# Codes4Fun/moshi.cpp

Measured on AMD Instinct MI355X. Metric: audio frames/sec (12.5 Hz target) moshika-7B q4_k decode, higher is better.
Workload: dtype q4_K weights x q8_K activations (int8 dot, f32 accumulate); bf16 KV; f32 elsewhere; 1 GPU; moshi-sts --bench loop: mimi encode + Temporal step + 8 Depth steps + mimi decode, moshika q4_k, 1 audio stream per GPU, greedy, ctx capacity 3000; context_fill_start=0, parallelism=1 GPU, device= (gfx950:sramecc+:xnack-)

## Files before the change

### include/ggml-backend.h

```cpp
#pragma once

#include "ggml.h"

#ifdef __cplusplus
extern "C" {
#endif

typedef struct ggml_backend_buffer_type * ggml_backend_buffer_type_t;
typedef struct ggml_backend_buffer      * ggml_backend_buffer_t;
typedef struct ggml_backend             * ggml_backend_t;
typedef struct ggml_backend_reg         * ggml_backend_reg_t;
typedef struct ggml_backend_device      * ggml_backend_dev_t;

enum ggml_backend_dev_type {
    GGML_BACKEND_DEVICE_TYPE_CPU,
    GGML_BACKEND_DEVICE_TYPE_GPU,
    GGML_BACKEND_DEVICE_TYPE_ACCEL,
};

struct ggml_backend_dev_caps {
    bool async;
    bool host_buffer;
    bool buffer_from_host_ptr;
    bool events;
};

struct ggml_backend_dev_props {
    const char * name;
    const char * description;
    size_t memory_free;
    size_t memory_total;
    enum ggml_backend_dev_type type;
    struct ggml_backend_dev_caps caps;
};

GGML_API void   ggml_backend_load_all(void);
GGML_API size_t ggml_backend_reg_count(void);
GGML_API ggml_backend_reg_t ggml_backend_reg_get(size_t index);
GGML_API const char * ggml_backend_reg_name(ggml_backend_reg_t reg);
GGML_API void * ggml_backend_reg_get_proc_address(ggml_backend_reg_t reg, const char * name);

GGML_API size_t             ggml_backend_dev_count(void);
GGML_API ggml_backend_dev_t ggml_backend_dev_get(size_t index);
GGML_API ggml_backend_dev_t ggml_backend_dev_by_name(const char * name);
GGML_API ggml_backend_dev_t ggml_backend_dev_by_type(enum ggml_backend_dev_type type);
GGML_API const char *       ggml_backend_dev_name(ggml_backend_dev_t device);
GGML_API const char *       ggml_backend_dev_description(ggml_backend_dev_t device);
GGML_API enum ggml_backend_dev_type ggml_backend_dev_type(ggml_backend_dev_t device);
GGML_API void               ggml_backend_dev_memory(ggml_backend_dev_t device, size_t * free, size_t * total);
GGML_API void               ggml_backend_dev_get_props(ggml_backend_dev_t device, struct ggml_backend_dev_props * props);
GGML_API ggml_backend_reg_t ggml_backend_dev_backend_reg(ggml_backend_dev_t device);
GGML_API ggml_backend_t     ggml_backend_dev_init(ggml_backend_dev_t device, const char * params);

GGML_API ggml_backend_t ggml_backend_init_by_name(const char * name, const char * params);
GGML_API ggml_backend_t ggml_backend_init_by_type(enum ggml_backend_dev_type type, const char * params);
GGML_API ggml_backend_t ggml_backend_init_best(void);

GGML_API const char *       ggml_backend_name(ggml_backend_t backend);
GGML_API void               ggml_backend_free(ggml_backend_t backend);
GGML_API ggml_backend_dev_t ggml_backend_get_device(ggml_backend_t backend);
GGML_API void               ggml_backend_synchronize(ggml_backend_t backend);

typedef void (*ggml_backend_set_n_threads_t)(ggml_backend_t backend, int n_threads);

GGML_API ggml_backend_buffer_t ggml_backend_alloc_ctx_tensors(struct ggml_context * ctx, ggml_backend_t backend);
GGML_API void    ggml_backend_buffer_free    (ggml_backend_buffer_t buffer);
GGML_API size_t  ggml_backend_buffer_get_size(ggml_backend_buffer_t buffer);
GGML_API void *  ggml_backend_buffer_get_base(ggml_backend_buffer_t buffer);
GGML_API const char * ggml_backend_buffer_name(ggml_backend_buffer_t buffer);
GGML_API void    ggml_backend_buffer_clear   (ggml_backend_buffer_t buffer, uint8_t value);
GGML_API bool    ggml_backend_buffer_is_host (ggml_backend_buffer_t buffer);

GGML_API void ggml_backend_tensor_set   (      struct ggml_tensor * tensor, const void * data, size_t offset, size_t size);
GGML_API void ggml_backend_tensor_get   (const struct ggml_tensor * tensor,       void * data, size_t offset, size_t size);
GGML_API void ggml_backend_tensor_get_async(ggml_backend_t backend, const struct ggml_tensor * tensor, void * data, size_t offset, size_t size);
typedef struct ggml_backend_event * ggml_backend_event_t;
GGML_API ggml_backend_event_t ggml_backend_event_new(ggml_backend_dev_t device);
GGML_API void ggml_backend_event_free(ggml_backend_event_t event);
GGML_API void ggml_backend_event_record(ggml_backend_event_t event, ggml_backend_t backend);
GGML_API void ggml_backend_event_synchronize(ggml_backend_event_t event);
GGML_API void ggml_backend_event_wait(ggml_backend_t backend, ggml_backend_event_t event);
GGML_API void ggml_backend_tensor_memset(      struct ggml_tensor * tensor, uint8_t value,     size_t offset, size_t size);
GGML_API void ggml_backend_tensor_copy  (struct ggml_tensor * src, struct ggml_tensor * dst);

GGML_API enum ggml_status ggml_backend_graph_compute(ggml_backend_t backend, struct ggml_cgraph * cgraph);
GGML_API bool ggml_backend_supports_op(ggml_backend_t backend, const struct ggml_tensor * op);

struct ggml_mi355x_stats {
    int64_t graphs_computed;
    int64_t graph_replays;
    int64_t kernels_in_last_plan;
    int64_t fused_nodes_in_last_plan;
    int64_t nodes_in_last_plan;
    int64_t uploads_batched;
    int64_t chained_matvecs_in_last_plan;
    int64_t attention_folds_planned;
    int64_t chain_step_programs_in_last_plan;
    int64_t vq_levels_chained_in_last_plan;
    int64_t attn_block_launches_in_last_plan;
    int64_t attn_block_jobs_in_last_plan;
    int64_t generic_attention_nodes_in_last_plan;
    int64_t ring_copy_launches_in_last_plan;
    int64_t ring_copy_jobs_in_last_plan;
};
GGML_API void ggml_backend_mi355x_get_stats(ggml_backend_t backend, struct ggml_mi355x_stats * stats);
struct ggml_mi355x_kernel_profile {
    double  seconds;
    int64_t launches;
    int64_t bytes;
    double  variant_seconds[3];
    int64_t variant_launches[3];
    int64_t variant_bytes[3];
    double  chain_seconds;
    int64_t chain_launches;
    int64_t chain_bytes;
    int64_t chain_phases;
};
GGML_API void ggml_backend_mi355x_get_kernel_profile(ggml_backend_t backend, struct ggml_mi355x_kernel_profile * out);
GGML_API void ggml_backend_mi355x_set_flags(ggml_backend_t backend, int flags);
GGML_API void ggml_backend_mi355x_set_capture(ggml_backend_t backend, int enabled);
GGML_API void * ggml_backend_mi355x_get_stream(ggml_backend_t backend);
GGML_API void ggml_backend_mi355x_make_current(ggml_backend_t backend);
GGML_API ggml_backend_t ggml_backend_mi355x_init_stream(ggml_backend_t base);

#ifdef __cplusplus
}
#endif
```

### moshi.cpp_amd/__init__.py

```python
import ctypes as C
import os

_HERE = os.path.dirname(os.path.abspath(__file__))
LIB_PATH = os.environ.get("MI355X_LIB") or os.path.join(_HERE, "libggml-mi355x.so")
HOT_LIB_PATH = os.environ.get("MI355X_HOT_LIB") or os.path.join(os.path.dirname(LIB_PATH), "libmoshi-hot.so")

GGML_MAX_DIMS, GGML_MAX_SRC, GGML_MAX_NAME = 4, 10, 64

F32, F16, Q4_0, Q8_0, Q4_K, Q8_K, I32, I64, BF16 = 0, 1, 2, 8, 12, 15, 26, 27, 30
TYPE_NAMES = {F32: "f32", F16: "f16", Q4_0: "q4_0", Q8_0: "q8_0", Q4_K: "q4_K", Q8_K: "q8_K", I32: "i32", I64: "i64", BF16: "bf16"}
DEV_CPU, DEV_GPU = 0, 1


class Tensor(C.Structure):
    pass


Tensor._fields_ = [
    ("type", C.c_int),
    ("buffer", C.c_void_p),
    ("ne", C.c_int64 * GGML_MAX_DIMS),
    ("nb", C.c_size_t * GGML_MAX_DIMS),
    ("op", C.c_int),
    ("op_params", C.c_int32 * 16),
    ("flags", C.c_int32),
    ("src", C.POINTER(Tensor) * GGML_MAX_SRC),
    ("view_src", C.POINTER(Tensor)),
    ("view_offs", C.c_size_t),
    ("data", C.c_void_p),
    ("name", C.c_char * GGML_MAX_NAME),
    ("extra", C.c_void_p),
    ("padding", C.c_char * 8),
]
TP = C.POINTER(Tensor)


class InitParams(C.Structure):
    _fields_ = [("mem_size", C.c_size_t), ("mem_buffer", C.c_void_p), ("no_alloc", C.c_bool)]


class DevProps(C.Structure):
    _fields_ = [("name", C.c_char_p), ("description", C.c_char_p), ("memory_free", C.c_size_t), ("memory_total", C.c_size_t),
                ("type", C.c_int), ("caps", C.c_bool * 4)]


class Stats(C.Structure):
    _fields_ = [(n, C.c_int64) for n in ("graphs_computed", "graph_replays", "kernels_in_last_plan",
                                         "fused_nodes_in_last_plan", "nodes_in_last_plan", "uploads_batched", "chained_matvecs_in_last_plan",
                                         "attention_folds_planned", "chain_step_programs_in_last_plan", "vq_levels_chained_in_last_plan",
                                         "attn_block_launches_in_last_plan", "attn_block_jobs_in_last_plan", "generic_attention_nodes_in_last_plan",
                                         "ring_copy_launches_in_last_plan", "ring_copy_jobs_in_last_plan")]


class KernelProfile(C.Structure):
    _fields_ = [("seconds", C.c_double), ("launches", C.c_int64), ("bytes", C.c_int64),
                ("variant_seconds", C.c_double * 3), ("variant_launches", C.c_int64 * 3), ("variant_bytes", C.c_int64 * 3),
                ("chain_seconds", C.c_double), ("chain_launches", C.c_int64), ("chain_bytes", C.c_int64), ("chain_phases", C.c_int64)]


class GGUFInitParams(C.Structure):
    _fields_ = [("no_alloc", C.c_bool), ("ctx", C.POINTER(C.c_void_p))]


P, I, L, Z, F, B, S = C.c_void_p, C.c_int, C.c_int64, C.c_size_t, C.c_float, C.c_bool, C.c_char_p

SIGNATURES = {
    "ggml_time_ms": (L, []), "ggml_time_us": (L, []), "ggml_time_init": (None, []),
    "ggml_type_name": (S, [I]), "ggml_op_name": (S, [I]), "ggml_op_desc": (S, [TP]), "ggml_status_to_string": (S, [I]),
    "ggml_blck_size": (L, [I]), "ggml_type_size": (Z, [I]), "ggml_row_size": (Z, [I, L]), "ggml_is_quantized": (B, [I]),
    "ggml_nelements": (L, [TP]), "ggml_nrows": (L, [TP]), "ggml_nbytes": (Z, [TP]), "ggml_element_size": (Z, [TP]),
    "ggml_n_dims": (I, [TP]), "ggml_is_contiguous": (B, [TP]), "ggml_is_transposed": (B, [TP]), "ggml_is_permuted": (B, [TP]),
    "ggml_are_same_shape": (B, [TP, TP]),
    "ggml_fp16_to_fp32": (F, [C.c_uint16]), "ggml_fp32_to_fp16": (C.c_uint16, [F]),
    "ggml_bf16_to_fp32": (F, [C.c_uint16]), "ggml_fp32_to_bf16": (C.c_uint16, [F]),
    "ggml_init": (P, [InitParams]), "ggml_reset": (None, [P]), "ggml_free": (None, [P]), "ggml_used_mem": (Z, [P]),
    "ggml_get_no_alloc": (B, [P]), "ggml_set_no_alloc": (None, [P, B]),
    "ggml_tensor_overhead": (Z, []), "ggml_graph_overhead": (Z, []), "ggml_graph_overhead_custom": (Z, [Z, B]),
    "ggml_new_tensor": (TP, [P, I, I, C.POINTER(L)]), "ggml_new_tensor_1d": (TP, [P, I, L]), "ggml_new_tensor_2d": (TP, [P, I, L, L]),
    "ggml_new_tensor_3d": (TP, [P, I, L, L, L]), "ggml_new_tensor_4d": (TP, [P, I, L, L, L, L]),
    "ggml_dup_tensor": (TP, [P, TP]), "ggml_view_tensor": (TP, [P, TP]),
    "ggml_get_first_tensor": (TP, [P]), "ggml_get_next_tensor": (TP, [P, TP]), "ggml_get_tensor": (TP, [P, S]),
    "ggml_get_name": (S, [TP]), "ggml_set_name": (TP, [TP, S]), "ggml_format_name": (TP, [TP, S]),
    "ggml_set_input": (None, [TP]), "ggml_set_output": (None, [TP]), "ggml_get_unary_op": (I, [TP]),
    "ggml_dup": (TP, [P, TP]), "ggml_add": (TP, [P, TP, TP]), "ggml_add_inplace": (TP, [P, TP, TP]), "ggml_sub": (TP, [P, TP, TP]),
    "ggml_sub_inplace": (TP, [P, TP, TP]), "ggml_mul_inplace": (TP, [P, TP, TP]), "ggml_div_inplace": (TP, [P, TP, TP]),
    "ggml_mul": (TP, [P, TP, TP]), "ggml_div": (TP, [P, TP, TP]), "ggml_neg": (TP, [P, TP]),
    "ggml_scale": (TP, [P, TP, F]), "ggml_scale_inplace": (TP, [P, TP, F]), "ggml_clamp": (TP, [P, TP, F, F]),
    "ggml_sum": (TP, [P, TP]), "ggml_sum_rows": (TP, [P, TP]), "ggml_argmax": (TP, [P, TP]),
    "ggml_argsort": (TP, [P, TP, I]), "ggml_argsort_top_k": (TP, [P, TP, I]), "ggml_top_k": (TP, [P, TP, I]),
    "ggml_arange": (TP, [P, F, F, F]), "ggml_repeat": (TP, [P, TP, TP]), "ggml_repeat_4d": (TP, [P, TP, L, L, L, L]),
    "ggml_concat": (TP, [P, TP, TP, I]), "ggml_pad": (TP, [P, TP, I, I, I, I]),
    "ggml_silu": (TP, [P, TP]), "ggml_gelu": (TP, [P, TP]), "ggml_elu": (TP, [P, TP]),
    "ggml_norm": (TP, [P, TP, F]), "ggml_rms_norm": (TP, [P, TP, F]), "ggml_mul_mat": (TP, [P, TP, TP]),
    "ggml_soft_max": (TP, [P, TP]), "ggml_soft_max_ext": (TP, [P, TP, TP, F, F]),
    "ggml_cast": (TP, [P, TP, I]), "ggml_cpy": (TP, [P, TP, TP]), "ggml_cont": (TP, [P, TP]),
    "ggml_reshape_1d": (TP, [P, TP, L]), "ggml_reshape_2d": (TP, [P, TP, L, L]), "ggml_reshape_3d": (TP, [P, TP, L, L, L]),
    "ggml_reshape_4d": (TP, [P, TP, L, L, L, L]),
    "ggml_view_1d": (TP, [P, TP, L, Z]), "ggml_view_2d": (TP, [P, TP, L, L, Z, Z]), "ggml_view_3d": (TP, [P, TP, L, L, L, Z, Z, Z]),
    "ggml_view_4d": (TP, [P, TP, L, L, L, L, Z, Z, Z, Z]),
    "ggml_permute": (TP, [P, TP, I, I, I, I]), "ggml_transpose": (TP, [P, TP]),
    "ggml_get_rows": (TP, [P, TP, TP]), "ggml_set_rows": (TP, [P, TP, TP, TP]),
    "ggml_im2col": (TP, [P, TP, TP, I, I, I, I, I, I, B, I]), "ggml_conv_1d": (TP, [P, TP, TP, I, I, I]),
    "ggml_conv_transpose_1d": (TP, [P, TP, TP, I, I, I]), "ggml_timestep_embedding": (TP, [P, TP, I, I]),
    "ggml_new_graph": (P, [P]), "ggml_new_graph_custom": (P, [P, Z, B]), "ggml_build_forward_expand": (None, [P, TP]),
    "ggml_graph_clear": (None, [P]), "ggml_graph_size": (I, [P]), "ggml_graph_n_nodes": (I, [P]), "ggml_graph_node": (TP, [P, I]),
    "ggml_graph_nodes": (C.POINTER(TP), [P]), "ggml_graph_n_leafs": (I, [P]), "ggml_graph_leaf": (TP, [P, I]), "ggml_graph_print": (None, [P]),
    "ggml_quantize_row": (None, [I, P, P, L]), "ggml_dequantize_row": (None, [I, P, P, L]),
    "ggml_backend_load_all": (None, []), "ggml_backend_reg_count": (Z, []), "ggml_backend_reg_get": (P, [Z]),
    "ggml_backend_reg_name": (S, [P]), "ggml_backend_reg_get_proc_address": (P, [P, S]),
    "ggml_backend_dev_count": (Z, []), "ggml_backend_dev_get": (P, [Z]), "ggml_backend_dev_by_name": (P, [S]),
    "ggml_backend_dev_by_type": (P, [I]), "ggml_backend_dev_name": (S, [P]), "ggml_backend_dev_description": (S, [P]),
    "ggml_backend_dev_type": (I, [P]), "ggml_backend_dev_memory": (None, [P, C.POINTER(Z), C.POINTER(Z)]),
    "ggml_backend_dev_get_props": (None, [P, C.POINTER(DevProps)]), "ggml_backend_dev_backend_reg": (P, [P]),
    "ggml_backend_dev_init": (P, [P, S]),
    "ggml_backend_init_by_name": (P, [S, S]), "ggml_backend_init_by_type": (P, [I, S]), "ggml_backend_init_best": (P, []),
    "ggml_backend_name": (S, [P]), "ggml_backend_free": (None, [P]), "ggml_backend_get_device": (P, [P]),
    "ggml_backend_synchronize": (None, [P]),
    "ggml_backend_alloc_ctx_tensors": (P, [P, P]), "ggml_backend_buffer_free": (None, [P]), "ggml_backend_buffer_get_size": (Z, [P]),
    "ggml_backend_buffer_get_base": (P, [P]), "ggml_backend_buffer_name": (S, [P]), "ggml_backend_buffer_clear": (None, [P, C.c_uint8]),
    "ggml_backend_buffer_is_host": (B, [P]),
    "ggml_backend_tensor_set": (None, [TP, P, Z, Z]), "ggml_backend_tensor_get": (None, [TP, P, Z, Z]),
    "ggml_backend_tensor_memset": (None, [TP, C.c_uint8, Z, Z]), "ggml_backend_tensor_copy": (None, [TP, TP]),
    "ggml_backend_graph_compute": (I, [P, P]), "ggml_backend_supports_op": (B, [P, TP]),
    "ggml_backend_mi355x_get_stats": (None, [P, C.POINTER(Stats)]), "ggml_backend_mi355x_set_flags": (None, [P, I]), "ggml_backend_mi355x_set_capture": (None, [P, I]),
    "ggml_backend_mi355x_get_stream": (P, [P]),
    "ggml_backend_mi355x_make_current": (None, [P]),
    "ggml_backend_mi355x_init_stream": (P, [P]),
    "ggml_backend_tensor_get_async": (None, [P, TP, P, Z, Z]),
    "ggml_backend_event_new": (P, [P]), "ggml_backend_event_free": (None, [P]), "ggml_backend_event_record": (None, [P, P]),
    "ggml_backend_event_synchronize": (None, [P]),
    "ggml_backend_event_wait": (None, [P, P]),
    "ggml_backend_mi355x_get_kernel_profile": (None, [P, C.POINTER(KernelProfile)]),
    "ggml_backend_cpu_init": (P, []), "ggml_backend_is_cpu": (B, [P]), "ggml_backend_cpu_set_n_threads": (None, [P, I]),
    "ggml_graph_compute_with_ctx": (I, [P, P, I]),
    "ggml_backend_cpu_reg": (P, []), "ggml_backend_cpu_set_graph_compute": (None, [P]),
    "gguf_init_empty": (P, []), "gguf_init_from_file": (P, [S, GGUFInitParams]), "gguf_free": (None, [P]),
    "gguf_get_version": (C.c_uint32, [P]), "gguf_get_alignment": (Z, [P]), "gguf_get_data_offset": (Z, [P]),
    "gguf_get_n_kv": (L, [P]), "gguf_find_key": (L, [P, S]), "gguf_get_key": (S, [P, L]), "gguf_get_val_str": (S, [P, L]),
    "gguf_get_val_u32": (C.c_uint32, [P, L]), "gguf_set_val_u32": (None, [P, S, C.c_uint32]), "gguf_set_val_str": (None, [P, S, S]),
    "gguf_get_n_tensors": (L, [P]), "gguf_find_tensor": (L, [P, S]), "gguf_get_tensor_name": (S, [P, L]),
    "gguf_get_tensor_type": (I, [P, L]), "gguf_get_tensor_offset": (Z, [P, L]), "gguf_get_tensor_size": (Z, [P, L]),
    "gguf_add_tensor": (None, [P, TP]), "gguf_write_to_file": (B, [P, S, B]),
}

_lib = None


class _Libs:

    def __init__(self, ggml, hot):
        self.ggml, self.hot = ggml, hot

    def __getattr__(self, name):
        for lib in (self.__dict__["ggml"], self.__dict__["hot"]):
            try:
                fn = getattr(lib, name)
            except AttributeError:
                continue
            setattr(self, name, fn)
            return fn
        raise AttributeError(name)


def load():
    global _lib
    if _lib is not None:
        return _lib
    for path in (LIB_PATH, HOT_LIB_PATH):
        if not os.path.exists(path):
            raise RuntimeError(f"{path} not found: build it with moshi.cpp_amd/build.sh (hipcc --offload-arch=gfx950); "
                               "there is no CPU or Python fallback for the decode hot path")
    lib = C.CDLL(LIB_PATH, mode=C.RTLD_GLOBAL)
    missing = []
    for name, (res, args) in SIGNATURES.items():
        try:
            fn = getattr(lib, name)
        except AttributeError:
            missing.append(name)
            continue
        fn.restype, fn.argtypes = res, args
    if missing:
        raise RuntimeError(f"libggml-mi355x.so lacks symbols declared in include/*.h: {missing}")
    stray = [n for n in ("moshi_hot_create", "moshi_hot_sts_frame") if hasattr(lib, n)]
    if stray:
        raise RuntimeError(f"the boundary library must not carry the harness: {stray}")
    hot_lib = C.CDLL(HOT_LIB_PATH, mode=C.RTLD_GLOBAL)
    from . import hot as _hot
    _hot.attach(hot_lib)
    _lib = _Libs(lib, hot_lib)
    return _lib


def declared_symbols():
    return sorted(SIGNATURES)
```

### moshi.cpp_amd/csrc/hip_attn_body.h

```cpp
#pragma once
#include "hip_device.h"

#define ATTN_NW_BASE 4
#define ATTN_NW_WIDE 8
#ifndef ATTN_SPLIT_NW_DEFAULT
#define ATTN_SPLIT_NW_DEFAULT 4
#endif
#define ATTN_MAX_T 4
#define ATTN_NPRE 4

struct attn_split_ws { unsigned long long * gscores; unsigned long long * gpart; unsigned * seq; int S; unsigned * err; int slots; int single_max; int big_min; };

#if defined(MV_LOG) && defined(ATTN_BODY_LOG)
#define AT_STAMP(i) do { if (blockIdx.x == 0 && blockIdx.y == 0 && threadIdx.x == 0) { if ((i) == 0) at_log_id = atomicAdd(&g_mv_launch, 1u) & 8191u; unsigned long long t_; asm volatile("s_memtime %0\n\ts_waitcnt lgkmcnt(0)" : "=s"(t_) :: "memory"); g_mv_log[at_log_id][i] = t_; \
    if ((i) == 0 || (i) == 7) { unsigned long long r_; asm volatile("s_memrealtime %0\n\ts_waitcnt lgkmcnt(0)" : "=s"(r_) :: "memory"); g_mv_log[at_log_id][16 + ((i) == 7)] = r_; } \
    if ((i) == 0) { g_mv_log[at_log_id][18] = (unsigned long long) a_in.D | ((unsigned long long) a_in.C << 32); g_mv_log[at_log_id][19] = 0xA7ull | ((unsigned long long) gridDim.x << 32); } } } while (0)
#else
#define AT_STAMP(i) do {} while (0)
#endif
#ifndef ATTN_V_EARLY
#define ATTN_V_EARLY 0
#endif
#define AT_PLAIN 0
#define AT_GQKV  2
#define AT_GOUT  4
struct attn_gqkv { const unsigned long long * in; int64_t qoff, koff, voff; unsigned * err; };
struct attn_gout { unsigned long long * out; unsigned tag; int64_t ts;
#if defined(CH_LOG)
                   unsigned long long * log;
#endif
};
#if defined(CH_LOG)
#define R256_STAMP(i) do { if (GOUT && go.log && threadIdx.x == 0) { unsigned long long t_; asm volatile("s_memrealtime %0\n\ts_waitcnt lgkmcnt(0)" : "=s"(t_) :: "memory"); go.log[i] = t_; } } while (0)
#else
#define R256_STAMP(i) do {} while (0)
#endif
template <bool SPLIT, int NWA, int MODE>
__device__ __forceinline__ void attn_decode_body(const attn_args & a_in, const attn_split_ws & w, char * smem, const int h, const int s_idx, const int group_y,
                                                 const unsigned gtag = 0u, const attn_gqkv gq = attn_gqkv(), const attn_gout go = attn_gout()) {
    constexpr bool GQKV = (MODE & AT_GQKV) != 0, GOUT = (MODE & AT_GOUT) != 0;
    constexpr int ATTN_NW = NWA, ATTN_THREADS = NWA * 64;
#if defined(MV_LOG)
    unsigned at_log_id = 0;
#endif
    AT_STAMP(0);
    attn_args a = a_in;
    if (!SPLIT && a.n_groups > 1) {
        const int t0 = 4 * group_y;
        a.T = a.T - t0 < 4 ? a.T - t0 : 4;
        a.q += (int64_t) t0 * a.q_ts; a.k += (int64_t) t0 * a.k_ts; a.v += (int64_t) t0 * a.v_ts;
        if (a.rot) a.rot += (int64_t) t0 * a.D;
        a.mask += (int64_t) t0 * a.C;
        a.index += t0;
        a.out += (int64_t) t0 * a.out_ts;
    }
    constexpr int NB = SPLIT ? (NWA == 8 ? 8 : 12) : ATTN_NPRE;
    constexpr int NPRE = ATTN_NPRE;
    const int D = SPLIT ? 128 : a.D, C = a.C, T = SPLIT ? 1 : a.T;
    const int S = SPLIT ? w.S : 1;
    int SLOTS = SPLIT ? w.slots : ATTN_SPLIT_SLOTS;
    int c_base = s_idx * SLOTS;
    const int tid = threadIdx.x, lane = tid & 63, wave = tid >> 6;
    float * sc   = (float *) smem;
    float * qf   = sc + C;
    float * knew = qf + T * D;
    float * vnew = knew + T * D;
    double * red = (double *) (smem + (((size_t) (C + 3 * T * D) * 4 + 15) & ~(size_t) 15));
    float * msk = (float *) (red + ATTN_NW * (64 / (D / 8)) * D);
    __shared__ float sh_f[ATTN_NW];
    __shared__ double sh_d[ATTN_NW];
    __shared__ int sh_i[ATTN_NW];
    __shared__ int sh_slot[ATTN_MAX_T];

    char * kc = a.kcache + (int64_t) h * a.k_nb2, * vc = a.vcache + (int64_t) h * a.v_nb2;
    const unsigned tag = SPLIT ? w.seq[h] + 1u : 0u;
    const int LPS = D / 8;
    const int SPW = 64 / LPS;
    const int sub = lane / LPS, dl = (lane % LPS) * 8;
    const int half = D / 2;

    auto scan_last_live = [&](int from) {
        int last = -1;
        if ((C & 3) == 0 && (from & 3) == 0 && (((uintptr_t) a.mask) & 15) == 0) {
            const int row4 = C / 4, from4 = from / 4, per_row = row4 - from4, n4 = T * per_row;
            for (int e0 = tid; e0 < n4; e0 += 3 * ATTN_THREADS) {
                float4 m4[3];
                int cs[3];
#pragma unroll
                for (int u = 0; u < 3; u++) {
                    const int e = e0 + u * ATTN_THREADS, ee = e < n4 ? e : n4 - 1;
                    const int t = ee / per_row, i4 = from4 + (ee - t * per_row);
                    cs[u] = i4 * 4;
                    m4[u] = ((const float4 *) a.mask)[t * row4 + i4];
                    if (e < n4) ((float4 *) msk)[t * row4 + i4] = m4[u];
                }
#pragma unroll
                for (int u = 0; u < 3; u++) {
                    if (e0 + u * ATTN_THREADS < n4) {
                        const int hi = m4[u].w > -INFINITY ? 3 : m4[u].z > -INFINITY ? 2 : m4[u].y > -INFINITY ? 1 : m4[u].x > -INFINITY ? 0 : -1;
                        if (hi >= 0) last = max(last, cs[u] + hi);
                    }
                }
            }
        } else {
            const int per_row = C - from;
            for (int e = tid; e < T * per_row; e += ATTN_THREADS) {
                const int t = e / per_row, c = from + (e - t * per_row);
                const float mv = a.mask[t * C + c];
                msk[t * C + c] = mv;
                if (mv > -INFINITY) last = max(last, c);
            }
        }
        return last;
    };
    auto block_max_i32 = [&](int v) {
        v = wave_allmax_i32(v);
        if (lane == 0) sh_i[wave] = v;
        __syncthreads();
        int r_ = sh_i[0];
#pragma unroll
        for (int w_ = 1; w_ < ATTN_NW; w_++) r_ = max(r_, sh_i[w_]);
        return r_;
    };

    int n_end = 0;
    if (MODE != AT_PLAIN && !SPLIT && s_idx > 0) return;
    if (SPLIT && s_idx > 0) {
        n_end = block_max_i32(scan_last_live(c_base)) + 1;
        if (n_end > w.big_min) { SLOTS *= 2; c_base = s_idx * SLOTS; }
        if (n_end <= w.single_max || n_end <= c_base) return;
        __syncthreads();
    }

    int slot_t[ATTN_MAX_T];
#pragma unroll
    for (int t = 0; t < ATTN_MAX_T; t++) slot_t[t] = a.index[t < T ? t : 0];
    float in_q0[2], in_q1[2], in_k0[2], in_k1[2], in_v[2], in_c[2], in_s[2];
#pragma unroll
    for (int u = 0; u < 2; u++) {
        const int e = tid + u * ATTN_THREADS;
        const int ee = e < T * D ? e : 0;
        const int t = ee / D, j = ee - t * D;
        const float * q = a.q + (int64_t) t * a.q_ts + (int64_t) h * a.q_hs;
        const float * k = a.k + (int64_t) t * a.k_ts + (int64_t) h * a.k_hs;
        const float * v = a.v + (int64_t) t * a.v_ts + (int64_t) h * a.v_hs;
        if (!GQKV) in_v[u] = v[j];
        if (a.rot) {
            const int p = j < half ? j : j - half;
            in_c[u] = a.rot[t * D + p]; in_s[u] = a.rot[t * D + half + p];
            if (!GQKV) { in_q0[u] = q[2 * p]; in_q1[u] = q[2 * p + 1]; in_k0[u] = k[2 * p]; in_k1[u] = k[2 * p + 1]; }
        } else {
            in_c[u] = 1.f; in_s[u] = 0.f;
            if (!GQKV) { in_q0[u] = q[j]; in_q1[u] = 0.f; in_k0[u] = k[j]; in_k1[u] = 0.f; }
        }
    }
    const bool scan_fast = (!SPLIT || s_idx == 0) && (C & 3) == 0 && (((uintptr_t) a.mask) & 15) == 0 && T * (C / 4) <= 3 * ATTN_THREADS;
    float4 m4pre[3];
    if (scan_fast) {
        const int row4 = C / 4, n4 = T * row4;
#pragma unroll
        for (int u = 0; u < 3; u++) { const int e = tid + u * ATTN_THREADS; m4pre[u] = ((const float4 *) a.mask)[e < n4 ? e : n4 - 1]; }
    }
    uint4 kpre[NPRE], vpre[NPRE];
#pragma unroll
    for (int pi = 0; pi < NPRE; pi++) {
        const int c = c_base + wave * SPW + pi * ATTN_NW * SPW + sub;
        const int cc = c < C ? c : C - 1;
        kpre[pi] = *(const uint4 *) (kc + (int64_t) cc * a.k_nb1 + dl * 2);
        if (pi < ATTN_NPRE) vpre[pi] = *(const uint4 *) (vc + (int64_t) cc * a.v_nb1 + dl * 2);
    }
    if (GQKV) {
#pragma unroll
        for (int u = 0; u < 2; u++) {
            const int e = tid + u * ATTN_THREADS;
            in_q0[u] = in_q1[u] = in_k0[u] = in_k1[u] = in_v[u] = 0.f;
            if (e < T * D) {
                const int t = e / D, j = e - t * D, p = j < half ? j : j - half;
                const int64_t eq = (int64_t) t * a.q_ts + (int64_t) h * a.q_hs, ek = (int64_t) t * a.k_ts + (int64_t) h * a.k_hs, ev = (int64_t) t * a.v_ts + (int64_t) h * a.v_hs;
                const unsigned long long * gp[5] = { gq.in + gq.qoff + eq + (a.rot ? 2 * p : j), gq.in + gq.qoff + eq + (a.rot ? 2 * p + 1 : j),
                                                     gq.in + gq.koff + ek + (a.rot ? 2 * p : j), gq.in + gq.koff + ek + (a.rot ? 2 * p + 1 : j), gq.in + gq.voff + ev + j };
                unsigned long long g[5];
                int spins = 0;
                for (;;) {
#pragma unroll
                    for (int i = 0; i < 5; i++) g[i] = __hip_atomic_load(gp[i], __ATOMIC_RELAXED, __HIP_MEMORY_SCOPE_AGENT);
                    bool ok = true;
#pragma unroll
                    for (int i = 0; i < 5; i++) ok = ok && (unsigned) (g[i] >> 32) == gtag;
                    if (ok) break;
                    if (++spins >= (1 << 20)) { if (gq.err) *gq.err = 5u; break; }
                    __builtin_amdgcn_s_sleep(1);
                }
                in_q0[u] = __uint_as_float((unsigned) g[0]); in_q1[u] = a.rot ? __uint_as_float((unsigned) g[1]) : 0.f;
                in_k0[u] = __uint_as_float((unsigned) g[2]); in_k1[u] = a.rot ? __uint_as_float((unsigned) g[3]) : 0.f;
                in_v[u] = __uint_as_float((unsigned) g[4]);
            }
        }
    }
    int last_live = -1;
    if (scan_fast) {
        const int row4 = C / 4, n4 = T * row4;
#pragma unroll
        for (int u = 0; u < 3; u++) {
            const int e = tid + u * ATTN_THREADS;
            if (e < n4) {
                ((float4 *) msk)[e] = m4pre[u];
                const int i4 = e % row4;
                const int hi = m4pre[u].w > -INFINITY ? 3 : m4pre[u].z > -INFINITY ? 2 : m4pre[u].y > -INFINITY ? 1 : m4pre[u].x > -INFINITY ? 0 : -1;
                if (hi >= 0) last_live = max(last_live, i4 * 4 + hi);
            }
        }
    } else if (!SPLIT || s_idx == 0) last_live = scan_last_live(0);
    __builtin_amdgcn_sched_barrier(0);
    AT_STAMP(1);

    if (tid < T) sh_slot[tid] = a.index[tid];
#pragma unroll
    for (int u = 0; u < 2; u++) {
        const int e = tid + u * ATTN_THREADS;
        if (e < T * D) {
            const int t = e / D, j = e - t * D;
            float qo, ko;
            if (a.rot) {
                if (j < half) { qo = in_q0[u] * in_c[u] - in_q1[u] * in_s[u]; ko = in_k0[u] * in_c[u] - in_k1[u] * in_s[u]; }
                else          { qo = in_q0[u] * in_s[u] + in_q1[u] * in_c[u]; ko = in_k0[u] * in_s[u] + in_k1[u] * in_c[u]; }
            } else { qo = in_q0[u]; ko = in_k0[u]; }
            const uint16_t kb = f2bf(ko), vb = f2bf(in_v[u]);
            qf[e] = bf2f(f2bf(qo));
            knew[e] = bf2f(kb);
            vnew[e] = bf2f(vb);
            const int slot = slot_t[t < ATTN_MAX_T ? t : 0];
            if (s_idx == 0 && (SPLIT || !a.row_split || group_y == 0) && slot >= 0 && slot < C) {
                ((uint16_t *) (kc + (int64_t) slot * a.k_nb1))[j] = kb;
                ((uint16_t *) (vc + (int64_t) slot * a.v_nb1))[j] = vb;
            }
        }
    }
    if (!SPLIT && a.write_only) return;
    if (!SPLIT || s_idx == 0) { n_end = block_max_i32(last_live) + 1; if (SPLIT && n_end > w.big_min) SLOTS *= 2; }
    else __syncthreads();
    AT_STAMP(2);
    const int P = SPLIT && n_end > w.single_max ? (n_end + SLOTS - 1) / SLOTS : 1;
    const bool multi = SPLIT && P > 1;
    const int c_lo = multi ? c_base : 0, c_hi = multi ? min(n_end, c_base + SLOTS) : n_end;
    const int c_last = c_hi > 0 ? c_hi - 1 : 0;
    auto pack_row = [&](const float * src) {
        float4 lo, hi;
        if ((C & 3) == 0) { lo = *(const float4 *) src; hi = *(const float4 *) (src + 4); }
        else { lo = make_float4(src[0], src[1], src[2], src[3]); hi = make_float4(src[4], src[5], src[6], src[7]); }
        uint4 r;
        r.x = (uint32_t) f2bf(lo.x) | ((uint32_t) f2bf(lo.y) << 16); r.y = (uint32_t) f2bf(lo.z) | ((uint32_t) f2bf(lo.w) << 16);
        r.z = (uint32_t) f2bf(hi.x) | ((uint32_t) f2bf(hi.y) << 16); r.w = (uint32_t) f2bf(hi.z) | ((uint32_t) f2bf(hi.w) << 16);
        return r;
    };
    auto fresh_of = [&](int c) { int f = -1; for (int tt = 0; tt < T; tt++) if (slot_t[tt] == c) f = tt; return f; };
#pragma unroll
    for (int pi = 0; pi < NPRE; pi++) {
        const int f = fresh_of(c_base + wave * SPW + pi * ATTN_NW * SPW + sub);
        if (f >= 0) { kpre[pi] = pack_row(knew + f * D + dl); if (pi < ATTN_NPRE) vpre[pi] = pack_row(vnew + f * D + dl); }
    }
    AT_STAMP(8);

    const int t_first = (!SPLIT && a.row_split) ? group_y : 0, t_last = (!SPLIT && a.row_split) ? group_y + 1 : T;
    for (int t = t_first; t < t_last; t++) {
        const float * mask = msk + t * C;
        float qv[8];
#pragma unroll
        for (int i = 0; i < 8; i++) qv[i] = qf[t * D + dl + i];
        AT_STAMP(9);
        float lmax = -INFINITY;
        auto score_pass = [&](int c0, const uint4 kv) {
            const int c = c0 + sub;
            const float m = c < c_hi ? mask[c] : -INFINITY;
            const bool live = m > -INFINITY;
            const uint32_t kw[4] = { kv.x, kv.y, kv.z, kv.w };
            double acc = 0;
#pragma unroll
            for (int i = 0; i < 4; i++) {
                acc += (double) (bf2f((uint16_t) (kw[i] & 0xffff)) * qv[2 * i]);
                acc += (double) (bf2f((uint16_t) (kw[i] >> 16)) * qv[2 * i + 1]);
            }
            acc = group_allsum_f64(acc, LPS);
            if (c < c_hi && (lane % LPS) == 0) {
                const float sv = live ? (float) acc * a.scale + m : -INFINITY;
                sc[c] = sv;
                lmax = fmaxf(lmax, sv);
            }
        };
        uint4 kb[NB];
        auto request_k_batch = [&](int cb) {
#pragma unroll
            for (int pi = 0; pi < NB; pi++) {
                const int c0 = cb + wave * SPW + pi * ATTN_NW * SPW, c = c0 + sub;
                kb[pi] = *(const uint4 *) (kc + (int64_t) (c < c_last ? c : c_last) * a.k_nb1 + dl * 2);
                if (SPLIT) __builtin_amdgcn_sched_barrier(0);
            }
        };
        const int cb_first = c_lo + NPRE * ATTN_NW * SPW;
#ifndef ATTN_LATE_ALWAYS
        const bool late_rows = SPLIT && cb_first < c_hi;
#else
        const bool late_rows = SPLIT;
#endif
        if (late_rows) request_k_batch(cb_first);
        uint4 vb0[SPLIT ? NB : 1];
        if (late_rows && ATTN_V_EARLY) {
#pragma unroll
            for (int pi = 0; pi < NB; pi++) {
                const int c0 = c_lo + (NPRE + pi) * ATTN_NW * SPW + wave * SPW, c = c0 + sub;
                vb0[pi] = *(const uint4 *) (vc + (int64_t) (c < c_last ? c : c_last) * a.v_nb1 + dl * 2);
                __builtin_amdgcn_sched_barrier(0);
            }
        }
#pragma unroll
        for (int pi = 0; pi < NPRE; pi++) {
            const int c0 = c_lo + wave * SPW + pi * ATTN_NW * SPW;
            if (c0 < c_hi) score_pass(c0, kpre[pi]);
        }
        for (int cb = cb_first; cb < c_hi; cb += NB * ATTN_NW * SPW) {
            if (!SPLIT || cb != cb_first) request_k_batch(cb);
#pragma unroll
            for (int pi = 0; pi < NB; pi++) {
                const int c0 = cb + wave * SPW + pi * ATTN_NW * SPW, f = fresh_of(c0 + sub);
                if (c0 < c_hi) {
                    if (f >= 0) kb[pi] = pack_row(knew + f * D + dl);
                    score_pass(c0, kb[pi]);
                }
            }
        }
        if (late_rows && !ATTN_V_EARLY) {
#pragma unroll
            for (int pi = 0; pi < NB; pi++) {
                const int c0 = c_lo + (NPRE + pi) * ATTN_NW * SPW + wave * SPW, c = c0 + sub;
                vb0[pi] = *(const uint4 *) (vc + (int64_t) (c < c_last ? c : c_last) * a.v_nb1 + dl * 2);
                __builtin_amdgcn_sched_barrier(0);
            }
        }
        AT_STAMP(10);
#ifndef ATTN_QUICK
#define ATTN_QUICK 1
#endif
        if (ATTN_QUICK && !multi && T == 1 && n_end <= 128 && n_end <= NPRE * ATTN_NW * SPW) {
            __syncthreads();
            AT_STAMP(3);
            const float s0 = lane < n_end ? sc[lane] : -INFINITY, s1 = lane + 64 < n_end ? sc[lane + 64] : -INFINITY;
            const float qmax = wave_allmax_f32(fmaxf(s0, s1));
            const float e0 = s0 > -INFINITY ? expf(s0 - qmax) : 0.f, e1 = s1 > -INFINITY ? expf(s1 - qmax) : 0.f;
            const double qsum = wave_allsum_f64((double) e0 + (double) e1);
            const float qinv = (float) (1.0 / qsum);
            AT_STAMP(4);
            double q8[8];
#pragma unroll
            for (int i = 0; i < 8; i++) q8[i] = 0;
#pragma unroll
            for (int pi = 0; pi < NPRE; pi++) {
                const int c0 = c_lo + wave * SPW + pi * ATTN_NW * SPW, c = c0 + sub;
                if (c0 < c_hi) {
                    const float sv = c < c_hi ? sc[c] : -INFINITY;
                    const float e = sv > -INFINITY ? expf(sv - qmax) : 0.f;
                    const float pq = c < c_hi ? bf2f(f2bf(e * qinv)) : 0.f;
                    const uint32_t vw[4] = { vpre[pi].x, vpre[pi].y, vpre[pi].z, vpre[pi].w };
#pragma unroll
                    for (int i = 0; i < 4; i++) {
                        q8[2 * i]     += (double) (bf2f((uint16_t) (vw[i] & 0xffff)) * pq);
                        q8[2 * i + 1] += (double) (bf2f((uint16_t) (vw[i] >> 16)) * pq);
                    }
                }
            }
            AT_STAMP(5);
#pragma unroll
            for (int i = 0; i < 8; i++) red[(wave * SPW + sub) * D + dl + i] = q8[i];
            __syncthreads();
            AT_STAMP(6);
            for (int j = lane; j < D; j += 64) {
                double tw = 0;
#pragma unroll
                for (int g = 0; g < 8; g++) if (g < SPW) tw += red[(wave * SPW + g) * D + j];
                red[(wave * SPW) * D + j] = tw;
            }
            __syncthreads();
            for (int j = tid; j < D; j += ATTN_THREADS) {
                double tot = 0;
#pragma unroll
                for (int w = 0; w < ATTN_NW; w++) tot += red[(w * SPW) * D + j];
                a.out[(int64_t) t * a.out_ts + (int64_t) h * D + j] = (float) tot;
                if (GOUT) __hip_atomic_store(go.out + (int64_t) t * go.ts + (int64_t) h * D + j, ((unsigned long long) go.tag << 32) | (unsigned long long) __float_as_uint((float) tot), __ATOMIC_RELAXED, __HIP_MEMORY_SCOPE_AGENT);
            }
            continue;
        }
        lmax = wave_allmax_f32(lmax);
        if (lane == 0) sh_f[wave] = lmax;
        AT_STAMP(11);
        __syncthreads();
        AT_STAMP(3);
        float gmax = sh_f[0];
#pragma unroll
        for (int w_ = 1; w_ < ATTN_NW; w_++) gmax = fmaxf(gmax, sh_f[w_]);
        if (multi) {
            {
                const int c = c_lo + tid;
                if (c < c_hi) __hip_atomic_store(w.gscores + (int64_t) h * C + c, ((unsigned long long) tag << 32) | (unsigned long long) __float_as_uint(sc[c]), __ATOMIC_RELAXED, __HIP_MEMORY_SCOPE_AGENT);
            }
            {
                constexpr int PULL = 3072 / ATTN_THREADS;
                float omax = -INFINITY;
                for (int c0 = tid; c0 < n_end; c0 += PULL * ATTN_THREADS) {
                    unsigned long long g[PULL];
                    int spins = 0;
                    for (;;) {
#pragma unroll
                        for (int u = 0; u < PULL; u++) {
                            const int c = c0 + u * ATTN_THREADS;
                            g[u] = __hip_atomic_load(w.gscores + (int64_t) h * C + (c < n_end ? c : n_end - 1), __ATOMIC_RELAXED, __HIP_MEMORY_SCOPE_AGENT);
                        }
                        bool ok = true;
#pragma unroll
                        for (int u = 0; u < PULL; u++) {
                            const int c = c0 + u * ATTN_THREADS;
                            if (c < n_end && (c < c_lo || c >= c_hi)) ok = ok && (unsigned) (g[u] >> 32) == tag;
                        }
                        if (ok) break;
                        if (++spins >= (1 << 20)) { if (w.err) *w.err = 1u; break; }
                        __builtin_amdgcn_s_sleep(1);
                    }
#pragma unroll
                    for (int u = 0; u < PULL; u++) {
                        const int c = c0 + u * ATTN_THREADS;
                        if (c < n_end && (c < c_lo || c >= c_hi)) { const float v = __uint_as_float((unsigned) g[u]); sc[c] = v; omax = fmaxf(omax, v); }
                    }
                }
                omax = wave_allmax_f32(omax);
                __syncthreads();
                if (lane == 0) sh_f[wave] = omax;
                __syncthreads();
#pragma unroll
                for (int w_ = 0; w_ < ATTN_NW; w_++) gmax = fmaxf(gmax, sh_f[w_]);
            }
        }

        double lsum = 0;
        for (int c = tid; c < n_end; c += ATTN_THREADS) {
            const float sv = sc[c];
            const float e = sv > -INFINITY ? expf(sv - gmax) : 0.f;
            sc[c] = e;
            lsum += (double) e;
        }
        lsum = wave_allsum_f64(lsum);
        if (lane == 0) sh_d[wave] = lsum;
        __syncthreads();
        double lall = sh_d[0];
#pragma unroll
        for (int w_ = 1; w_ < ATTN_NW; w_++) lall += sh_d[w_];
        const float inv = (float) (1.0 / lall);
        AT_STAMP(4);

        double o8[8];
#pragma unroll
        for (int i = 0; i < 8; i++) o8[i] = 0;
        auto pv_pass = [&](int c0, const uint4 vv) {
            const int c = c0 + sub;
            const float p = c < c_hi ? bf2f(f2bf(sc[c] * inv)) : 0.f;
            const uint32_t vw[4] = { vv.x, vv.y, vv.z, vv.w };
#pragma unroll
            for (int i = 0; i < 4; i++) {
                o8[2 * i]     += (double) (bf2f((uint16_t) (vw[i] & 0xffff)) * p);
                o8[2 * i + 1] += (double) (bf2f((uint16_t) (vw[i] >> 16)) * p);
            }
        };
#pragma unroll
// ... 364 lines not shown
```

### moshi.cpp_amd/csrc/hip_backend.hip

```cpp
#include "hip_common.h"
#include "ggml-cpu.h"

#include <string.h>

#include <algorithm>
#include <functional>
#include <deque>
#include <map>
#include <memory>
#include <set>
#include <string>
#include <unordered_map>
#include <vector>

#define UPLOAD_SLOTS       8
#define UPLOAD_BLOB_BYTES  (64 * 1024)
#define UPLOAD_MAX_DESCS   1024
#define READBACK_PINNED_BYTES (64 * 1024)
#define AGET_SLOTS 64
#define AGET_SLOT_BYTES 256
#define UPLOAD_SMALL_MAX   16384

struct plan_t;

struct upload_slot {
    char * blob = nullptr;
    upload_desc * descs = nullptr;
    hipEvent_t done = nullptr;
    bool in_flight = false;
};

struct hip_ctx {
    int device = 0;
    std::string name, description;
    hipStream_t stream = nullptr;
    int flags = 0;
    bool no_capture = false;
    ggml_mi355x_stats stats = {};
    std::map<size_t, std::vector<void *>> pool;
    upload_slot slots[UPLOAD_SLOTS];
    int cur_slot = 0;
    int n_pending = 0;
    size_t pending_bytes = 0;
    mv_profile prof = { nullptr, 0, 0 };
    double prof_seconds = 0; int64_t prof_launches = 0, prof_bytes = 0;
    double prof_seconds_v[3] = { 0, 0, 0 }; int64_t prof_launches_v[3] = { 0, 0, 0 }, prof_bytes_v[3] = { 0, 0, 0 };
    double prof_chain_seconds = 0; int64_t prof_chain_launches = 0, prof_chain_bytes = 0, prof_chain_phases = 0;
    hipEvent_t chain_ev[2] = { nullptr, nullptr };
    std::unordered_map<const ggml_cgraph *, plan_t *> plans;
    uint64_t orphan_clock = 0;
    volatile unsigned * err_host = nullptr;
    unsigned * err_dev = nullptr;
    char * readback = nullptr;
    struct async_get { void * dst; size_t size; int slot; uint64_t seq; };
    char * aget_pinned = nullptr;
    std::deque<async_get> aget_pending;
    uint64_t aget_seq = 0;
    bool in_use = false;
    int usable_cus = 0;
    ggml_backend_device dev_obj;
};

static std::vector<hip_ctx *> & contexts() { static std::vector<hip_ctx *> v; return v; }
static std::vector<hip_ctx *> & stream_contexts() { static std::vector<hip_ctx *> v; return v; }

static void set_device(hip_ctx * c) { HIP_CHECK(hipSetDevice(c->device)); }

static void ctx_init_lazy(hip_ctx * c) {
    if (c->stream) return;
    set_device(c);
    {
        hipDeviceProp_t prop;
        HIP_CHECK(hipGetDeviceProperties(&prop, c->device));
        c->usable_cus = prop.multiProcessorCount;
        const char * e = getenv("MI355X_STREAM_CUS");
        const int lim = e ? atoi(e) : 0;
        if (lim > 0 && lim < prop.multiProcessorCount) {
            std::vector<uint32_t> mask((size_t) (prop.multiProcessorCount + 31) / 32, 0u);
            for (int i = 0; i < lim; i++) mask[(size_t) i / 32] |= 1u << (i % 32);
            HIP_CHECK(hipExtStreamCreateWithCUMask(&c->stream, (uint32_t) mask.size(), mask.data()));
            c->usable_cus = lim;
        }
    }
    if (!c->stream) HIP_CHECK(hipStreamCreateWithFlags(&c->stream, hipStreamNonBlocking));
    for (auto & s : c->slots) {
        HIP_CHECK(hipHostMalloc((void **) &s.blob, UPLOAD_BLOB_BYTES, hipHostMallocMapped));
        HIP_CHECK(hipHostMalloc((void **) &s.descs, UPLOAD_MAX_DESCS * sizeof(upload_desc), hipHostMallocMapped));
        HIP_CHECK(hipEventCreateWithFlags(&s.done, hipEventDisableTiming));
    }
    HIP_CHECK(hipHostMalloc((void **) &c->readback, READBACK_PINNED_BYTES, hipHostMallocDefault));
    HIP_CHECK(hipHostMalloc((void **) &c->aget_pinned, AGET_SLOTS * AGET_SLOT_BYTES, hipHostMallocDefault));
    HIP_CHECK(hipHostMalloc((void **) &c->err_host, 64, hipHostMallocMapped));
    c->err_host[0] = 0u;
    HIP_CHECK(hipHostGetDevicePointer((void **) &c->err_dev, (void *) c->err_host, 0));
}

static void check_device_error(hip_ctx * c) {
    if (c->err_host && c->err_host[0] != 0u)
        GGML_ABORT("mi355x backend: a kernel gave up a bounded wait (code %u: 1 = split attention head barrier, 2 = chain engine hand-off, 3 = stream engine hand-off); results are invalid", c->err_host[0]);
}

static size_t size_class(size_t n) {
    if (n > ((size_t) 64 << 20)) return 0;
    size_t c = 256;
    while (c < n) c <<= 1;
    return c;
}
static void * pool_poison(hip_ctx * c, void * p, size_t n) {
    static const bool poison = getenv("MI355X_POISON") != nullptr;
    if (poison && p) { HIP_CHECK(hipMemsetAsync(p, 0xFF, n, c->stream)); HIP_CHECK(hipStreamSynchronize(c->stream)); }
    return p;
}
#define GUARD_BYTES 4096
static bool guard_mode() { static const bool g = getenv("MI355X_GUARD") != nullptr; return g; }
static void guard_fill(hip_ctx * c, char * user, size_t actual) {
    HIP_CHECK(hipMemsetAsync(user - GUARD_BYTES, 0xA5, GUARD_BYTES, c->stream));
    HIP_CHECK(hipMemsetAsync(user + actual, 0xA5, GUARD_BYTES, c->stream));
}
static void guard_check(hip_ctx * c, char * user, size_t actual) {
    static std::vector<unsigned char> h(2 * GUARD_BYTES);
    HIP_CHECK(hipStreamSynchronize(c->stream));
    HIP_CHECK(hipMemcpy(h.data(), user - GUARD_BYTES, GUARD_BYTES, hipMemcpyDeviceToHost));
    HIP_CHECK(hipMemcpy(h.data() + GUARD_BYTES, user + actual, GUARD_BYTES, hipMemcpyDeviceToHost));
    for (size_t i = 0; i < 2 * GUARD_BYTES; i++)
        if (h[i] != 0xA5) GGML_ABORT("mi355x: guard zone %s a %zu-byte allocation was overwritten (offset %zu)", i < GUARD_BYTES ? "before" : "after", actual, i % GUARD_BYTES);
}
static void * pool_alloc(hip_ctx * c, size_t n, size_t * actual) {
    set_device(c);
    const size_t cls = size_class(n ? n : 1);
    if (cls) {
        auto & fl = c->pool[cls];
        *actual = cls;
        if (!fl.empty()) { void * p = fl.back(); fl.pop_back(); if (guard_mode()) guard_fill(c, (char *) p, *actual); return pool_poison(c, p, *actual); }
    } else *actual = n;
    void * p = nullptr;
// ... 1741 lines not shown
        for (int i = 0; i < g->n_nodes && !no_lowrank; i++) {
            const ggml_tensor * mm = g->nodes[i];
            if (an.skip[(size_t) i] || mm->op != GGML_OP_MUL_MAT || mm->type != GGML_TYPE_F32) continue;
            const ggml_tensor * W = mm->src[0], * gr = mm->src[1];
            if (W->type != GGML_TYPE_Q8_0 || !dense_rows(W) || W->ne[2] * W->ne[3] != 1 || gr->op != GGML_OP_GET_ROWS || gr->type != GGML_TYPE_F32) continue;
            const int pg = pos_of(an, gr);
            if (pg < 0 || an.skip[(size_t) pg] || uses_of(an, gr) != 1 || ggml_nelements(gr) != gr->ne[0] || gr->ne[0] != W->ne[0]) continue;
            const ggml_tensor * tab = gr->src[0], * idx = gr->src[1];
            if (ggml_nelements(idx) != 1 || idx->type != GGML_TYPE_I32 || !dense_rows(tab) || !idx->data) continue;
            switch (tab->type) { case GGML_TYPE_F32: case GGML_TYPE_F16: case GGML_TYPE_BF16: case GGML_TYPE_Q4_0: case GGML_TYPE_Q8_0: break; default: continue; }
            const int64_t K = W->ne[0], M = W->ne[1];
            if (K % 32 != 0 || K > 2048 || ggml_nelements(mm) != M || !ggml_is_contiguous(mm)) continue;
            std::vector<int> members = { pg, i };
            float * out = (float *) mm->data;
            int emit = i;
            const ggml_tensor * cp = sole_consumer(an, mm);
            if (cp && cp->op == GGML_OP_CPY && uses_of(an, mm) == 1 && cp->type == GGML_TYPE_F32 && cp->src[0] == mm && ggml_is_contiguous(cp) && cp->view_src == NULL &&
                ggml_are_same_shape(cp, mm) && pos_of(an, cp) >= 0 && !an.skip[(size_t) pos_of(an, cp)]) {
                members.push_back(pos_of(an, cp)); out = (float *) cp->data; emit = pos_of(an, cp);
            }
            for (int m2 : members) an.skip[(size_t) m2] = 1;
            const lowrank_embed_args la = { (const char *) tab->data, (int64_t) tab->nb[1], tab->ne[1], (int) tab->type, (const int32_t *) idx->data,
                                            (const char *) W->data, (int64_t) W->nb[1], (int) K, (int) M, out };
            p->lowrank_copies.emplace_back(new lowrank_embed_args(la));
            at_pos[emit].push_back(pstep::special_step([=](hipStream_t s) { k_lowrank_embed(s, la); }, 2, nullptr, p->lowrank_copies.back().get()));
            p->n_fused += (int) members.size();
        }
        for (int i = g->n_nodes - 1; i >= 0; i--) {
            if (an.skip[(size_t) i] || g->nodes[i]->op != GGML_OP_ADD) continue;
            embed_group grp;
            if (!match_embed_sum(an, i, grp)) continue;
            bool clash = false;
            for (int m : grp.members) if (m < 0 || an.skip[(size_t) m]) clash = true;
            if (clash) continue;
            for (int m : grp.members) an.skip[(size_t) m] = 1;
            const embed_sum_args a = grp.a;
            at_pos[i].push_back([=](hipStream_t s) { k_embed_sum(s, a); });
            p->n_fused += (int) grp.members.size();
        }
        for (int i = 0; i < g->n_nodes; i++) {
            row_copy_group rg;
            if (an.skip[(size_t) i] || g->nodes[i]->op != GGML_OP_CONT || !match_row_copies(an, i, rg)) continue;
            for (int m : rg.members) an.skip[(size_t) m] = 1;
            const copy_rows_args ra = rg.a;
            at_pos[rg.emit_pos].push_back([=](hipStream_t s) { k_copy_rows(s, ra); });
            p->n_fused += (int) rg.members.size();
        }
        for (int i = 0; i < g->n_nodes; i++) {
            const ggml_tensor * n = g->nodes[i];
            if (an.skip[(size_t) i] || n->op != GGML_OP_CPY) continue;
            const ggml_tensor * ct = n->src[0];
            const int pc = pos_of(an, ct);
            if (ct->op != GGML_OP_CONT || pc < 0 || an.skip[(size_t) pc] || uses_of(an, ct) != 1 || ct->view_src) continue;
            if (ct->type != GGML_TYPE_F32 || n->type != GGML_TYPE_F32 || ct->src[0]->type != GGML_TYPE_F32 || !ggml_are_same_shape(ct, ct->src[0]) ||
                !ggml_are_same_shape(n, ct) || !ggml_is_contiguous(n)) continue;
            bool writer_between = false;
            for (int j = pc + 1; j < i; j++) if (writes_through_alias(g->nodes[j])) writer_between = true;
            if (writer_between) continue;
            an.skip[(size_t) i] = an.skip[(size_t) pc] = 1;
            const tdesc d = make_tdesc(n), x = make_tdesc(ct->src[0]);
            at_pos[i].push_back([=](hipStream_t s) { k_cpy(s, d, x); });
            p->n_fused += 2;
        }
        for (int i = 0; i < g->n_nodes; i++) {
            const ggml_tensor * n = g->nodes[i];
            if (an.skip[(size_t) i] || n->op != GGML_OP_TIMESTEP_EMBEDDING) continue;
            const ggml_tensor * ad = n->src[0];
            const int pa = pos_of(an, ad);
            if (ad->op != GGML_OP_ADD || pa < 0 || an.skip[(size_t) pa] || uses_of(an, ad) != 1 || ad->view_src || ad->type != GGML_TYPE_F32) continue;
            const ggml_tensor * x = ad->src[0], * y = ad->src[1];
            if (x->type != GGML_TYPE_F32 || y->type != GGML_TYPE_F32 || !ggml_is_contiguous(x) || !ggml_is_contiguous(y) || !ggml_are_same_shape(x, ad) ||
                ggml_nelements(ad) != ad->ne[0] || !(ggml_nelements(y) == ggml_nelements(ad) || ggml_nelements(y) == 1)) continue;
            an.skip[(size_t) i] = an.skip[(size_t) pa] = 1;
            const tdesc d = make_tdesc(n), tx = make_tdesc(x);
            const float * yp = (const float *) y->data; const int yn = (int) ggml_nelements(y);
            const int dim = n->op_params[0], mp = n->op_params[1];
            {
                pstep st([=](hipStream_t s) { k_timestep_embedding(s, d, tx, dim, mp, yp, yn); });
                if (x->op == GGML_OP_NONE && y->op == GGML_OP_NONE && !x->view_src && !y->view_src) { st.hoist_dst = (const char *) n->data; st.hoist_bytes = ggml_nbytes(n); }
                at_pos[i].push_back(std::move(st));
            }
            p->n_fused += 2;
        }
        std::unordered_map<const void *, float *> paired_gate;
        size_t paired_consumed = 0;
        static const bool no_pair = getenv("MI355X_PAIRED_GATE") != nullptr && atoi(getenv("MI355X_PAIRED_GATE")) == 0;
        static const bool no_batched_fusion = getenv("MI355X_NO_BATCHED_MM") != nullptr || getenv("MI355X_NO_BATCHED_FUSION") != nullptr;
        for (int i = 0; i < g->n_nodes; i++) {
            if (an.skip[(size_t) i] || g->nodes[i]->op != GGML_OP_MUL_MAT) continue;
            mv_group grp;
            if (!match_matvec(an, i, grp)) {
                bmm_group bg;
                if (!no_batched_fusion && match_batched_mm(an, i, em, bg)) {
                    bool bclash = false;
                    for (int m : bg.members) if (m != i && an.skip[(size_t) m]) bclash = true;
                    if (!bclash) {
                        for (int m : bg.members) an.skip[(size_t) m] = 1;
                        at_pos[bg.emit_pos].push_back(bg.run);
                        p->n_fused += (int) bg.members.size();
                    }
                }
                continue;
            }
            bool clash = false;
            for (int m : grp.members) if (m < 0 || (m != i && an.skip[(size_t) m])) clash = true;
            if (clash) continue;
            for (int m : grp.members) an.skip[(size_t) m] = 1;
            mv_args a = grp.a;
            if (is_qblock((enum ggml_type) a.wtype) && a.ncols == 1 && !no_argmax_epilogue) {
                const ggml_tensor * ynode = g->nodes[grp.emit_pos];
                const ggml_tensor * am = nullptr;
                int n_am = 0;
                for (int j = grp.emit_pos + 1; j < g->n_nodes; j++) if (g->nodes[j]->op == GGML_OP_ARGMAX && g->nodes[j]->src[0] == ynode) { am = g->nodes[j]; n_am++; }
                if (am && n_am == 1 && !an.skip[(size_t) pos_of(an, am)] && (float *) ynode->data == a.y && ggml_nelements(ynode) == a.M && am->data) {
                    a.argmax_out[0] = (int32_t *) am->data;
                    an.skip[(size_t) pos_of(an, am)] = 1;
                    const ggml_tensor * cp = nullptr;
                    for (int j = pos_of(an, am) + 1; j < g->n_nodes; j++)
                        if (g->nodes[j]->op == GGML_OP_CPY && g->nodes[j]->src[0] == am && g->nodes[j]->type == GGML_TYPE_I32 && ggml_nelements(g->nodes[j]) == 1) { cp = g->nodes[j]; break; }
                    if (cp && !an.skip[(size_t) pos_of(an, cp)]) { a.argmax_out[1] = (int32_t *) cp->data; an.skip[(size_t) pos_of(an, cp)] = 1; }
                    unsigned * tk = (unsigned *) em.ws(256 + 2 * 4 * 8192);
                    HIP_CHECK(hipMemsetAsync(tk, 0, 256, em.c->stream));
                    a.ticket = tk;
                    p->n_fused += 1 + (cp ? 1 : 0);
                }
            }
            if (a.prologue == MV_PLAIN && is_qblock((enum ggml_type) a.wtype) && a.ncols == 1 && !no_attn_prologue) {
                for (auto & ag : attn_groups) {
                    const attn_args & at = ag.a;
                    if (ag.emit_pos < 0 || ag.B > 1 || ag.column || (const float *) at.out != a.x || at.T != 1 || at.D != 64 || at.C > 8 || (int64_t) at.H * at.D != a.K) continue;
                    if (a.K != 1024 || at.H != 16 || ag.emit_pos > grp.emit_pos || uses_of(an, g->nodes[ag.emit_pos]) != 1) continue;
                    p->attn_copies.emplace_back(new attn_args(at));
                    a.prologue = MV_ATTN;
                    a.attn = p->attn_copies.back().get();
                    ag.emit_pos = -1;
                    break;
                }
            }
            if (a.prologue == MV_RMSNORM && a.wtype == GGML_TYPE_Q4_K && a.ncols == 1 && keep && !(c->flags & 512) && grp.emit_pos == i) {
                bool merged = false;
                for (auto & ag : attn_groups) {
                    const attn_args & at = ag.a;
                    if (ag.emit_pos < 0 || ag.B > 1 || ag.column || at.q != a.y || ag.emit_pos < grp.emit_pos) continue;
                    if (!k_inproj_attn_supported(a, at, c->usable_cus)) continue;
                    bool private_y = true;
                    std::vector<const ggml_tensor *> aliases { g->nodes[i] };
                    for (int j = i + 1; j < g->n_nodes && private_y; j++) {
                        const ggml_tensor * nj = g->nodes[j];
                        bool reads = false;
                        for (int sidx = 0; sidx < GGML_MAX_SRC; sidx++)
                            if (nj->src[sidx] && std::find(aliases.begin(), aliases.end(), nj->src[sidx]) != aliases.end()) reads = true;
                        if (!reads) continue;
                        const bool layout = nj->op == GGML_OP_VIEW || nj->op == GGML_OP_RESHAPE || nj->op == GGML_OP_PERMUTE || nj->op == GGML_OP_TRANSPOSE;
                        if (layout) { aliases.push_back(nj); continue; }
                        if (std::find(ag.members.begin(), ag.members.end(), j) == ag.members.end()) private_y = false;
                    }
                    if (!private_y || !spin_kernels_allowed(c)) continue;
                    const mv_args am = a; const attn_args aa = at;
                    unsigned * err = c->err_dev;
                    const size_t wn = k_inproj_attn_ws_size(a, at);
                    void * ws = em.ws(wn);
                    HIP_CHECK(hipMemsetAsync(ws, 0, wn, c->stream));
                    at_pos[ag.emit_pos].insert(at_pos[ag.emit_pos].begin(), [=](hipStream_t s) { k_inproj_attn(s, am, aa, ws, err); });
                    ag.emit_pos = -1;
                    p->n_fused += 1; p->n_attn_folded++; c->stats.attention_folds_planned++;
                    merged = true;
                    break;
                }
                if (merged) { if (grp.members.size() > 1) p->n_fused += (int) grp.members.size(); continue; }
            }
            if (!no_pair && a.prologue != MV_GATE_SILU && a.ncols == 1 && a.residual == nullptr && a.res_embed.table == nullptr && a.ticket == nullptr &&
                a.M % 2 == 0 && k_matvec_pair_ok(a.wtype, a.K, a.M / 2) && grp.emit_pos == i) {
                const ggml_tensor * h = g->nodes[i];
                const int64_t F = a.M / 2;
                const ggml_tensor * l = nullptr, * r = nullptr;
                int nv = 0;
                for (int j = i + 1; j < g->n_nodes && j < i + 12; j++) {
                    const ggml_tensor * v = g->nodes[j];
                    if (v->op == GGML_OP_VIEW && v->src[0] == h) { nv++; if (v->data == h->data) l = v; else if ((const char *) v->data == (const char *) h->data + F * 4) r = v; }
                }
                if (uses_of(an, h) == 2 && nv == 2 && l && r && ggml_nelements(l) == F && ggml_nelements(r) == F && ggml_is_contiguous(l) && ggml_is_contiguous(r) &&
                    uses_of(an, l) == 1 && uses_of(an, r) == 1) {
                    const ggml_tensor * sl = sole_consumer(an, l), * ml = sole_consumer(an, r);
                    if (sl && sl->op == GGML_OP_UNARY && sl->op_params[0] == GGML_UNARY_OP_SILU && uses_of(an, sl) == 1 && ml && ml->op == GGML_OP_MUL &&
                        ml->src[0] == sl && ml->src[1] == r && uses_of(an, ml) == 1) {
                        const ggml_tensor * mo = sole_consumer(an, ml);
                        bool consumer_ok = false;
                        if (mo && mo->op == GGML_OP_MUL_MAT && mo->src[1] == ml && is_qblock(mo->src[0]->type) && mo->src[0]->ne[0] == F && F > 4096 &&
                            !an.skip[(size_t) pos_of(an, mo)]) {
                            mv_group cg;
                            const int mpos = pos_of(an, mo);
                            consumer_ok = match_matvec(an, mpos, cg) && cg.a.prologue == MV_GATE_SILU && (const void *) cg.a.x == h->data && cg.a.K == F && cg.a.ncols == 1;
                            for (int m2 : cg.members) if (m2 < 0 || (m2 != mpos && an.skip[(size_t) m2])) consumer_ok = false;
                        }
                        if (consumer_ok) {
                            float * gbuf = (float *) em.ws((size_t) F * 4);
                            a.pair_F = F;
                            a.y = gbuf;
                            paired_gate[h->data] = gbuf;
                        }
                    }
                }
            }
            if (a.prologue == MV_GATE_SILU && is_qblock((enum ggml_type) a.wtype) && a.K > 4096 && paired_gate.count((const void *) a.x)) {
                const float * gbuf = paired_gate[(const void *) a.x];
                paired_consumed++;
                a.prologue = MV_PLAIN;
                a.x = gbuf;
                a.x_cs = a.K;
            }
            if (a.prologue == MV_GATE_SILU && is_qblock((enum ggml_type) a.wtype) && a.K > 4096) {
                void * blocks = em.ws((size_t) (a.K / 256) * MV_XBLK_BYTES);
                const float * h = a.x; const int64_t K = a.K;
                const int wt = a.wtype;
                at_pos[grp.emit_pos].push_back([=](hipStream_t s) { k_gate_quant_q8k(s, h, K, blocks, wt); });
                a.prologue = MV_PREQ8K;
                a.x = (const float *) blocks;
            }
            at_pos[grp.emit_pos].push_back(pstep(a));
            if (grp.members.size() > 1) p->n_fused += (int) grp.members.size();
        }
        GGML_ASSERT(paired_consumed == paired_gate.size() && "a linear_in was redirected to the paired gate form but its linear_out did not pick the gate vector up");
    }
    if (fuse) {
        for (int i = 0; i < g->n_nodes; i++) {
            const ggml_tensor * nn = g->nodes[i];
            if (an.skip[(size_t) i] || (nn->op != GGML_OP_NORM && nn->op != GGML_OP_RMS_NORM) || nn->type != GGML_TYPE_F32 || ggml_nelements(nn) != nn->ne[0] || uses_of(an, nn) != 1) continue;
            if (nn->src[0]->type != GGML_TYPE_F32 || nn->src[0]->nb[0] != 4) continue;
            const ggml_tensor * ml = sole_consumer(an, nn);
            if (!ml || ml->op != GGML_OP_MUL || ml->view_src || pos_of(an, ml) < 0 || an.skip[(size_t) pos_of(an, ml)]) continue;
            const ggml_tensor * wv = ml->src[0] == nn ? ml->src[1] : ml->src[0];
            if (wv == nn || wv->type != GGML_TYPE_F32 || !ggml_is_contiguous(wv) || ggml_nelements(wv) != nn->ne[0] || !wv->data || !ggml_is_contiguous(ml)) continue;
            std::vector<int> members = { i, pos_of(an, ml) };
            const ggml_tensor * last = ml; const float * bp = nullptr;
            const ggml_tensor * ad = uses_of(an, ml) == 1 ? sole_consumer(an, ml) : nullptr;
            if (ad && ad->op == GGML_OP_ADD && !ad->view_src && pos_of(an, ad) >= 0 && !an.skip[(size_t) pos_of(an, ad)] && ggml_is_contiguous(ad)) {
                const ggml_tensor * bv = ad->src[0] == ml ? ad->src[1] : ad->src[0];
                if (bv != ml && bv->type == GGML_TYPE_F32 && ggml_is_contiguous(bv) && ggml_nelements(bv) == nn->ne[0] && bv->data && bv->op == GGML_OP_NONE && ad->src[0] == ml) {
                    bp = (const float *) bv->data; last = ad; members.push_back(pos_of(an, ad));
                }
            }
            for (int m2 : members) an.skip[(size_t) m2] = 1;
            const tdesc a = make_tdesc(nn->src[0]); const float eps = ggml_get_op_params_f32(nn, 0); const int rms = nn->op == GGML_OP_RMS_NORM;
            const float * wp = (const float *) wv->data; float * out = (float *) last->data;
            at_pos[pos_of(an, last)].push_back([=](hipStream_t s) { k_norm_affine(s, a, eps, rms, wp, bp, out); });
            p->n_fused += (int) members.size();
        }
    }
    for (size_t gi = 0; gi < attn_groups.size(); ) {
        if (!attn_groups[gi].column || attn_groups[gi].emit_pos < 0) { gi++; continue; }
        const attn_args & a0 = attn_groups[gi].a;
        std::set<int> inside(attn_groups[gi].members.begin(), attn_groups[gi].members.end());
        size_t ge = gi + 1;
        int lo = attn_groups[gi].emit_pos, hi = lo;
        const attn_args * rows = a0.T > 1 ? &a0 : nullptr;
        while (ge < attn_groups.size() && ge - gi < ATTN_BLOCKS_MAX) {
            const attn_group & n = attn_groups[ge];
            const attn_args & b = n.a;
            if (!n.column || n.emit_pos < 0 || b.H != a0.H || b.D != a0.D || b.C != a0.C || b.scale != a0.scale || b.out_ts != a0.out_ts || (b.rot != nullptr) != (a0.rot != nullptr) ||
                (b.T > 1 && rows && (b.q_ts != rows->q_ts || b.k_ts != rows->k_ts || b.v_ts != rows->v_ts)) || b.q_hs != a0.q_hs || b.k_hs != a0.k_hs || b.v_hs != a0.v_hs ||
                b.k_nb1 != a0.k_nb1 || b.k_nb2 != a0.k_nb2 || b.v_nb1 != a0.v_nb1 || b.v_nb2 != a0.v_nb2 || b.kcache == a0.kcache) break;
            std::set<int> both = inside;
            both.insert(n.members.begin(), n.members.end());
            const int nlo = n.emit_pos < lo ? n.emit_pos : lo, nhi = n.emit_pos > hi ? n.emit_pos : hi;
            bool clean = true;
            for (int i = nlo + 1; i < nhi && clean; i++) if (!is_view_op(g->nodes[i]->op) && !both.count(i)) clean = false;
            if (!clean) break;
            inside.swap(both); lo = nlo; hi = nhi;
            if (b.T > 1 && !rows) rows = &b;
            ge++;
        }
        attn_blocks_args ba;
        memset(&ba, 0, sizeof(ba));
        ba.a = a0;
        if (rows) { ba.a.q_ts = rows->q_ts; ba.a.k_ts = rows->k_ts; ba.a.v_ts = rows->v_ts; }
        ba.n_jobs = (int) (ge - gi);
        for (size_t k = gi; k < ge; k++) {
            const attn_args & b = attn_groups[k].a;
            ba.job[k - gi] = { b.q, b.k, b.v, b.kcache, b.vcache, b.mask, b.rot, b.index, b.out, b.T };
            attn_groups[k].emit_pos = -1;
        }
        unsigned * err = c->err_dev;
        auto & at = at_pos[hi];
        at.insert(at.begin(), [=](hipStream_t s) { attn_blocks_args b = ba; b.write_only = 0; k_attn_blocks(s, b, err); });
        at.insert(at.begin(), [=](hipStream_t s) { attn_blocks_args b = ba; b.write_only = 1; k_attn_blocks(s, b, err); });
// ... 261 lines not shown
    }
    flush_uploads(c);
    h->c = c; h->seq = c->aget_seq;
    HIP_CHECK(hipEventRecord(h->ev, c->stream));
}
static void hip_event_wait(ggml_backend_t b, ggml_backend_event_t e) {
    hip_ctx * c = (hip_ctx *) b->context;
    hip_event_ctx * h = (hip_event_ctx *) e->context;
    if (!h) return;
    ctx_init_lazy(c);
    set_device(c);
    flush_uploads(c);
    HIP_CHECK(hipStreamWaitEvent(c->stream, h->ev, 0));
}
static bool hip_supports_op(ggml_backend_t, const struct ggml_tensor * op) {
    switch (op->op) {
        case GGML_OP_CPY: case GGML_OP_CONT: case GGML_OP_DUP:
            if (ggml_is_quantized(op->type) || ggml_is_quantized(op->src[0]->type)) {
                if (op->type == op->src[0]->type) return true;
                const enum ggml_type st = op->src[0]->type;
                return (st == GGML_TYPE_F32 || st == GGML_TYPE_F16 || st == GGML_TYPE_BF16) &&
                       (op->type == GGML_TYPE_Q8_0 || op->type == GGML_TYPE_Q4_0 || op->type == GGML_TYPE_Q4_K) && op->src[0]->ne[0] % ggml_blck_size(op->type) == 0;
            }
            return true;
        case GGML_OP_MUL_MAT:
            switch (op->src[0]->type) { case GGML_TYPE_F32: case GGML_TYPE_F16: case GGML_TYPE_BF16: case GGML_TYPE_Q4_0: case GGML_TYPE_Q8_0: case GGML_TYPE_Q4_K: return true; default: return false; }
        default: return op->op < GGML_OP_COUNT;
    }
}

static const char * hip_dev_name(ggml_backend_dev_t d) { return ((hip_ctx *) d->context)->name.c_str(); }
static const char * hip_dev_desc(ggml_backend_dev_t d) { return ((hip_ctx *) d->context)->description.c_str(); }
static void hip_dev_memory(ggml_backend_dev_t d, size_t * free, size_t * total) {
    hip_ctx * c = (hip_ctx *) d->context;
    set_device(c);
    if (hipMemGetInfo(free, total) != hipSuccess) { *free = 0; *total = 0; }
}
static enum ggml_backend_dev_type hip_dev_type(ggml_backend_dev_t) { return GGML_BACKEND_DEVICE_TYPE_GPU; }
static ggml_backend_t hip_dev_init(ggml_backend_dev_t d, const char *) {
    hip_ctx * c = (hip_ctx *) d->context;
    ctx_init_lazy(c);
    if (c->flags != 0) { HIP_CHECK(hipStreamSynchronize(c->stream)); for (auto & kv : c->plans) plan_free(c, kv.second); c->plans.clear(); c->flags = 0; }
    c->stats = {};
    auto * b = new ggml_backend;
    b->iface = { hip_backend_name, hip_backend_free, hip_backend_sync, hip_alloc_buffer, hip_graph_compute, hip_supports_op, hip_get_tensor_async, hip_event_record, hip_event_wait };
    b->device = d;
    b->context = c;
    return b;
}

static const char * hip_reg_name(ggml_backend_reg_t) { return "ROCm"; }
static size_t hip_reg_dev_count(ggml_backend_reg_t) { return contexts().size(); }
static ggml_backend_dev_t hip_reg_get_dev(ggml_backend_reg_t, size_t i) { return &contexts()[i]->dev_obj; }
static void * hip_reg_proc(ggml_backend_reg_t, const char *) { return NULL; }

extern "C" ggml_backend_reg_t ggml_backend_mi355x_reg(void) {
    static ggml_backend_reg reg = { { hip_reg_name, hip_reg_dev_count, hip_reg_get_dev, hip_reg_proc }, NULL };
    static bool init = false;
    if (!init) {
        init = true;
        int n = 0;
        if (hipGetDeviceCount(&n) != hipSuccess) n = 0;
        for (int i = 0; i < n; i++) {
            hipDeviceProp_t prop;
            if (hipGetDeviceProperties(&prop, i) != hipSuccess) continue;
            hip_ctx * c = new hip_ctx;
            c->device = i;
            c->name = "ROCm" + std::to_string(i);
            c->description = std::string(prop.name) + " (" + prop.gcnArchName + ")";
            c->dev_obj.iface = { hip_dev_name, hip_dev_desc, hip_dev_memory, hip_dev_type, hip_dev_init };
            c->dev_obj.reg = &reg;
            c->dev_obj.context = c;
            contexts().push_back(c);
        }
    }
    return contexts().empty() ? NULL : &reg;
}

static hip_ctx * ctx_of(ggml_backend_t b) {
    GGML_ASSERT(b && b->iface.get_name == hip_backend_name && "not an MI355X backend");
    return (hip_ctx *) b->context;
}
extern "C" void ggml_backend_mi355x_get_stats(ggml_backend_t b, struct ggml_mi355x_stats * stats) { *stats = ctx_of(b)->stats; }
extern "C" void ggml_backend_mi355x_set_capture(ggml_backend_t b, int enabled) {
    if (b && b->iface.get_name == hip_backend_name) ((hip_ctx *) b->context)->no_capture = !enabled;
}
extern "C" void ggml_backend_mi355x_set_flags(ggml_backend_t b, int flags) {
    hip_ctx * c = ctx_of(b);
    if (c->stream) { flush_uploads(c); HIP_CHECK(hipStreamSynchronize(c->stream)); }
    for (auto & kv : c->plans) plan_free(c, kv.second);
    c->plans.clear();
    c->flags = flags;
}
extern "C" void ggml_backend_mi355x_get_kernel_profile(ggml_backend_t b, struct ggml_mi355x_kernel_profile * out) {
    hip_ctx * c = ctx_of(b);
    out->seconds = c->prof_seconds; out->launches = c->prof_launches; out->bytes = c->prof_bytes;
    for (int v = 0; v < 3; v++) { out->variant_seconds[v] = c->prof_seconds_v[v]; out->variant_launches[v] = c->prof_launches_v[v]; out->variant_bytes[v] = c->prof_bytes_v[v]; }
    out->chain_seconds = c->prof_chain_seconds; out->chain_launches = c->prof_chain_launches; out->chain_bytes = c->prof_chain_bytes; out->chain_phases = c->prof_chain_phases;
}
extern "C" void * ggml_backend_mi355x_get_stream(ggml_backend_t b) { hip_ctx * c = ctx_of(b); ctx_init_lazy(c); return (void *) c->stream; }
extern "C" void ggml_backend_mi355x_make_current(ggml_backend_t b) { hip_ctx * c = ctx_of(b); ctx_init_lazy(c); set_device(c); }
extern "C" ggml_backend_t ggml_backend_mi355x_init_stream(ggml_backend_t base) {
    if (!base || base->iface.get_name != hip_backend_name) return NULL;
    hip_ctx * b0 = (hip_ctx *) base->context;
    hip_ctx * c = nullptr;
    int n_same = 0;
    for (hip_ctx * o : stream_contexts()) if (o->device == b0->device) { n_same++; if (!o->in_use && !c) c = o; }
    if (!c) {
        c = new hip_ctx;
        c->device = b0->device;
        c->name = b0->name + "/s" + std::to_string(n_same + 1);
        c->description = b0->description + ", additional stream";
        c->dev_obj.iface = b0->dev_obj.iface;
        c->dev_obj.reg = b0->dev_obj.reg;
        c->dev_obj.context = c;
        stream_contexts().push_back(c);
    }
    c->in_use = true;
    ggml_backend_t b = c->dev_obj.iface.init_backend(&c->dev_obj, NULL);
    c->flags = b0->flags;
    c->no_capture = b0->no_capture;
    return b;
}
```

### moshi.cpp_amd/csrc/hip_common.h

```cpp
#pragma once

#include <hip/hip_runtime.h>
#include <stdint.h>

#include "ggml_impl.h"

#define HIP_CHECK(expr) do { hipError_t e_ = (expr); if (e_ != hipSuccess) \
    GGML_ABORT("HIP error %s at %s: %s", hipGetErrorName(e_), #expr, hipGetErrorString(e_)); } while (0)

struct tdesc {
    char *  data;
    int64_t ne[4];
    int64_t nb[4];
    int     type;
};

static inline tdesc make_tdesc(const struct ggml_tensor * t) {
    tdesc d;
    d.data = (char *) t->data;
    for (int i = 0; i < 4; i++) { d.ne[i] = t->ne[i]; d.nb[i] = (int64_t) t->nb[i]; }
    d.type = (int) t->type;
    return d;
}

static inline int64_t td_nelements(const tdesc & t) { return t.ne[0] * t.ne[1] * t.ne[2] * t.ne[3]; }

void k_binary(hipStream_t s, int op, tdesc dst, tdesc a, tdesc b);
void k_unary(hipStream_t s, int uop, tdesc dst, tdesc a);
void k_scale(hipStream_t s, tdesc dst, tdesc a, float scale, float bias);
void k_clamp(hipStream_t s, tdesc dst, tdesc a, float mn, float mx);
void k_cpy(hipStream_t s, tdesc dst, tdesc src);
void k_concat(hipStream_t s, tdesc dst, tdesc a, tdesc b, int dim);
void k_repeat(hipStream_t s, tdesc dst, tdesc a);
void k_pad(hipStream_t s, tdesc dst, tdesc a);
void k_arange(hipStream_t s, tdesc dst, float start, float step);
void k_sum_rows(hipStream_t s, tdesc dst, tdesc a);
void k_sum_all(hipStream_t s, tdesc dst, tdesc a);
void k_argmax(hipStream_t s, tdesc dst, tdesc a);
void k_argsort(hipStream_t s, tdesc dst, tdesc a, int desc);
void k_norm(hipStream_t s, tdesc dst, tdesc a, float eps, int rms);
void k_norm_affine(hipStream_t s, tdesc a, float eps, int rms, const float * w, const float * b, float * out);
void k_soft_max(hipStream_t s, tdesc dst, tdesc a, tdesc mask, int has_mask, float scale);
void k_get_rows(hipStream_t s, tdesc dst, tdesc a, tdesc idx);
void k_set_rows(hipStream_t s, tdesc dst, tdesc src, tdesc idx);
void k_im2col(hipStream_t s, tdesc dst, tdesc x, int64_t K, int s0, int p0, int d0);
size_t k_conv_transpose_1d_ws_size(const struct ggml_tensor * w, const struct ggml_tensor * x);
void k_conv_transpose_1d(hipStream_t s, tdesc dst, tdesc w, tdesc x, int s0, void * ws);
void k_timestep_embedding(hipStream_t s, tdesc dst, tdesc ts, int dim, int max_period, const float * addend = nullptr, int addend_n = 0);
size_t k_mul_mat_ws_size(const struct ggml_tensor * a, const struct ggml_tensor * b);
struct conv_scatter { uint16_t * panel; const float * prev; int K, Kw, s0, TP, M, C, elu, pad; };
struct mm_epilogue { const float * bias; const char * residual; int64_t res_nb0, res_nb1;
                     float * tail_prev; int tail_TP, tail_pre_elu, tail_L, tail_C; const char * tail_x; int64_t tail_nb0, tail_nb1;
                     conv_scatter sc;
                     const char * af_x; int64_t af_nb0, af_nb1; int af_elu, af_pad; };
void k_mul_mat(hipStream_t s, tdesc dst, tdesc a, tdesc b, void * ws, const mm_epilogue * epi = nullptr);
bool k_mul_mat_is_few_rows(tdesc a, tdesc b);
void k_stream_im2col(hipStream_t s, tdesc dst, const float * prev, int TP, tdesc x, int Kw, int s0, int pre_elu);
void k_conv_tail(hipStream_t s, float * prev, int TP, tdesc x, int pre_elu);
void k_convtr_finish(hipStream_t s, tdesc out, float * prev, const float * bias, const void * ws, int K, int OC, int L, int s0, int nsplit, const conv_scatter * sc = nullptr);
void k_dw_convtr_frame(hipStream_t s, float * out, float * prev, const float * bias, const char * x, int64_t x_cs, const char * w, int64_t w_cs, int K, int PT, int C, int64_t out_cs = -1, int64_t out_ks = 1);
int  k_conv_transpose_1d_partial(hipStream_t s, tdesc w, tdesc x, void * ws, int pre_elu);
struct upload_desc { char * dst; uint32_t offset; uint32_t size; };
void k_scatter_uploads(hipStream_t s, const upload_desc * descs, const char * blob, int n);

enum mv_prologue { MV_PLAIN = 0, MV_RMSNORM = 1, MV_GATE_SILU = 2, MV_LAYERNORM = 3, MV_GELU = 4, MV_PREQ8K = 5, MV_ATTN = 6 };
struct attn_args;
struct embed_src { const char * table; int64_t row_bytes; int64_t n_rows; int type; const int32_t * index; const float * scale; };
#define MV_MAX_COLS 4
struct mv_args {
    int         wtype;
    const char * w;
    int64_t     row_bytes;
    int64_t     K, M;
    int         prologue;
    const float * x;
    const float * alpha;
    const float * beta;
    float       eps;
    int         ncols;
    int64_t     x_cs, y_cs, r_cs;
    int         out_act;
    const float * out_scale;
    const float * residual;
    float *     y;
    float *     x_out;
    embed_src   res_embed;
    int32_t *   argmax_out[2];
    unsigned *  ticket;
    const attn_args * attn;
    int64_t     pair_F;
    int         special;
    const struct lowrank_embed_args * lr;
    const struct sample_args * smp;
};
struct chain_plan;
bool   k_chain_default_on();
int    k_chain_accept(const mv_args * mv, int n, int usable_cus, bool allow_step_program = true);
size_t k_chain_ws_size(const mv_args * mv, int n, int usable_cus, bool allow_step_program = true);
chain_plan * k_chain_create(hipStream_t s, const mv_args * mv, int n, void * ws, unsigned * err, int usable_cus, bool allow_step_program);
bool   k_chain_is_step_program(const chain_plan * c);
void   k_chain_launch(hipStream_t s, const chain_plan * c);
void   k_chain_free(chain_plan * c);
int    k_chain_length(const chain_plan * c);
int64_t k_chain_weight_bytes(const chain_plan * c);
bool k_matvec_supported(int wtype, int64_t K, int64_t M);
bool k_matvec_pair_ok(int wtype, int64_t K, int64_t F);
struct mv_profile {
    struct rec { hipEvent_t start, stop; int64_t bytes; int variant; };
    rec * recs; int capacity; int used;
};
void k_matvec_set_profile(mv_profile * p);
void k_matvec(hipStream_t s, const mv_args & a);
#define MV_XBLK_BYTES 304
void k_gate_quant_q8k(hipStream_t s, const float * h, int64_t K, void * out_blocks, int wtype);
void k_norm_quant_q8k(hipStream_t s, const float * x, const float * alpha, float eps, int64_t K, void * out_blocks, int wtype, float * n_out);
size_t k_mm_q4k_batched_ws_size(int64_t K, int64_t T);
bool k_mm_q4k_batched_supported(int wtype, int64_t K, int64_t M, int64_t T);
void k_mm_q4k_batched(hipStream_t s, int wtype, const char * w, int64_t row_bytes, int64_t K, int64_t M, int64_t T, const float * x, int64_t x_cs,
                      void * ws, float * y, int64_t y_cs, const float * residual, int64_t r_cs, int prologue = 0, const float * alpha = nullptr, float eps = 0.f);

struct attn_args {
    const float * q; const float * k; const float * v;
    int64_t q_ts, q_hs, k_ts, k_hs, v_ts, v_hs;
    const float * rot;
    const float * mask;
    const int32_t * index;
    char * kcache; char * vcache;
    int64_t k_nb1, k_nb2, v_nb1, v_nb2;
    int H, D, C, T;
    float scale;
    float * out;
    int64_t out_ts;
    int n_groups, write_only;
    int row_split;
};
#define ATTN_SPLIT_MIN_C 1024
#define ATTN_SPLIT_SLOTS 128
#define ATTN_SPLIT_BIG_MIN 1024
#define ATTN_SINGLE_MAX 384
size_t k_attn_decode_ws_size(const attn_args & a);
bool k_attn_split_resident(const attn_args & a, int usable_cus);
void k_attn_decode(hipStream_t s, const attn_args & a, void * ws = nullptr, unsigned * err = nullptr);
struct attn_streams_args { attn_args a; int B; int64_t q_bs, k_bs, v_bs, kc_bs, vc_bs, out_bs, mask_bs, rot_bs, index_bs; };
void k_attn_streams(hipStream_t s, const attn_streams_args & a, unsigned * err = nullptr);
#define ATTN_BLOCKS_MAX 16
struct attn_block_job { const float * q, * k, * v; char * kcache, * vcache; const float * mask, * rot; const int32_t * index; float * out; int T; };
struct attn_blocks_args { attn_args a; int n_jobs, write_only; attn_block_job job[ATTN_BLOCKS_MAX]; };
void k_attn_blocks(hipStream_t s, const attn_blocks_args & a, unsigned * err = nullptr);
#define COPY_ROWS_MAX 16
struct copy_rows_args { const float * src[COPY_ROWS_MAX]; float * dst; int64_t n; int rows; };
void k_copy_rows(hipStream_t s, const copy_rows_args & a);
#define RING_COPY_MAX 64
struct ring_copy_job { const char * src; char * dst; int64_t src_hs, dst_hs; };
struct ring_copy_args { int n_jobs, H; int64_t run_bytes; int blocks_per_run; ring_copy_job job[RING_COPY_MAX]; };
void k_ring_copy(hipStream_t s, const ring_copy_args & a, int usable_cus);

bool   k_inproj_attn_supported(const mv_args & a, const attn_args & at, int usable_cus);
size_t k_inproj_attn_ws_size(const mv_args & a, const attn_args & at);
void   k_inproj_attn(hipStream_t s, const mv_args & a, const attn_args & at, void * ws, unsigned * err);

struct xattn_args { const float * q; const char * k; const char * v; int64_t k_nb1, k_nb2, v_nb1, v_nb2; int H, D, Tc; float scale; float * out; };
void k_cross_attn(hipStream_t s, const xattn_args & a);

#define EMBED_SUM_MAX 40
struct embed_sum_args { embed_src src[EMBED_SUM_MAX]; int n; int64_t K; float * out; int B; };
void k_embed_sum(hipStream_t s, const embed_sum_args & a);
struct vq_level_args {
    const char * emb; int64_t emb_row_bytes; int D, NC;
    const char * resid; int64_t resid_stride;
    const float * add_c; const float * num;
    float * resid_out; float * idx_f; int32_t * idx_i;
    float * cand_val; int32_t * cand_idx; unsigned * counter;
};
#define GATHER_MAX 32
struct gather_args { const float * src[GATHER_MAX]; int n; void * dst; int dst_type; };
void k_gather_scalars(hipStream_t s, const gather_args & a);
#define SAMPLE_MAX_N 32768
#define SAMPLE_MAX_K 256
struct lowrank_embed_args { const char * table; int64_t row_bytes, n_rows; int type; const int32_t * index; const char * w; int64_t w_row_bytes; int K, M; float * out; };
void k_lowrank_embed(hipStream_t s, const lowrank_embed_args & a);
struct sample_args { const float * logits; int n; float scale; int k; const float * noise; int32_t * out; int32_t * out2; };
void k_sample_topk(hipStream_t s, const sample_args & a);
#define SAMPLE_MAX_B 16
struct sample_streams_args { const float * logits; int n; float scale; const float * inv_temp; int k; const float * noise; int32_t * out; int32_t * out2; int B; };
void k_sample_topk_streams(hipStream_t s, const sample_streams_args & a);
#define VQ_LEVEL_WS_BYTES 4096
void k_vq_level(hipStream_t s, const vq_level_args & a);
struct vq_chain_plan;
bool   k_vq_chain_accept(const vq_level_args * lv, int n, int usable_cus);
size_t k_vq_chain_ws_size(int n);
vq_chain_plan * k_vq_chain_create(hipStream_t s, const vq_level_args * lv, int n, void * ws, unsigned * err);
void   k_vq_chain_launch(hipStream_t s, const vq_chain_plan * c);
void   k_vq_chain_free(vq_chain_plan * c);
```

### moshi.cpp_amd/csrc/hip_kernels_fused.hip

```cpp
#include "hip_common.h"
#include "hip_device.h"
#include "hip_mv_device.h"
#include <hip/hip_ext.h>
#include <stdlib.h>
#include <map>

struct x_src {
    int prologue;
    const float * x;
    const float * alpha;
    float scale;
    int64_t K;
};

__device__ __forceinline__ float x_value(const x_src & s, int64_t i) {
    switch (s.prologue) {
        case MV_RMSNORM:   return s.alpha[i] * (s.x[i] * s.scale);
        case MV_GATE_SILU: { const float l = s.x[i], r = s.x[s.K + i]; return (l / (1.0f + expf(-l))) * r; }
        default:           return s.x[i];
    }
}

__device__ float block_rms_scale(const float * x, int64_t K, float eps, double * sh) {
    double acc = 0;
// ... 114 lines not shown
            if (j < half) { qo = qr[hh] * rc - qi[hh] * rs; ko = kr[hh] * rc - ki[hh] * rs; }
            else          { qo = qr[hh] * rs + qi[hh] * rc; ko = kr[hh] * rs + ki[hh] * rc; }
        } else { qo = qr[hh]; ko = kr[hh]; }
        const uint16_t kb = f2bf(ko), vb = f2bf(vv[hh]);
        float * wb = wbuf + hh * 192;
        wb[j] = bf2f(f2bf(qo)); wb[64 + j] = bf2f(kb); wb[128 + j] = bf2f(vb);
        if (write_cache && slot >= 0 && slot < C) {
            const int h = h0 + hh;
            ((uint16_t *) (a.kcache + (int64_t) h * a.k_nb2 + (int64_t) slot * a.k_nb1))[j] = kb;
            ((uint16_t *) (a.vcache + (int64_t) h * a.v_nb2 + (int64_t) slot * a.v_nb1))[j] = vb;
        }
    }
    __builtin_amdgcn_fence(__ATOMIC_RELEASE, "wavefront");
    __builtin_amdgcn_wave_barrier();
    __builtin_amdgcn_fence(__ATOMIC_ACQUIRE, "wavefront");
    float * prod = wbuf + 768;
#pragma unroll
    for (int hp = 0; hp < NH; hp += 2) {
#pragma unroll
        for (int hq = 0; hq < 2; hq++) {
            const int hh = hp + hq;
            const float * qf = wbuf + hh * 192, * knew = qf + 64, * vnew = qf + 128;
            float qv[8];
#pragma unroll
            for (int i = 0; i < 8; i++) qv[i] = qf[dl + i];
            double acc = 0;
            if (live) {
                if (fresh) {
#pragma unroll
                    for (int i = 0; i < 8; i++) acc += (double) (knew[dl + i] * qv[i]);
                } else {
                    const uint32_t kw[4] = { kq[hh].x, kq[hh].y, kq[hh].z, kq[hh].w };
#pragma unroll
                    for (int i = 0; i < 4; i++) {
                        acc += (double) (bf2f((uint16_t) (kw[i] & 0xffff)) * qv[2 * i]);
                        acc += (double) (bf2f((uint16_t) (kw[i] >> 16)) * qv[2 * i + 1]);
                    }
                }
            }
            acc = group_allsum_f64(acc, LPS);
            const float sv = live ? (float) acc * a.scale + m : -INFINITY;
            const float gmax = wave_allmax_f32(sv);
            const float e = sv > -INFINITY ? expf(sv - gmax) : 0.f;
            double lsum = (lane % LPS) == 0 ? (double) e : 0.0;
            lsum = wave_allsum_f64(lsum);
            const float inv = (float) (1.0 / lsum);
            const float pr = bf2f(f2bf(e * inv));
            float pf[8];
#pragma unroll
            for (int i = 0; i < 8; i++) pf[i] = 0.f;
            if (pr != 0.f) {
                if (fresh) {
#pragma unroll
                    for (int i = 0; i < 8; i++) pf[i] = vnew[dl + i] * pr;
                } else {
                    const uint32_t vw[4] = { vq[hh].x, vq[hh].y, vq[hh].z, vq[hh].w };
#pragma unroll
                    for (int i = 0; i < 4; i++) {
                        pf[2 * i]     = bf2f((uint16_t) (vw[i] & 0xffff)) * pr;
                        pf[2 * i + 1] = bf2f((uint16_t) (vw[i] >> 16)) * pr;
                    }
                }
            }
            float * dst = prod + hq * 512 + sub * 64 + dl;
            *(float4 *) dst = make_float4(pf[0], pf[1], pf[2], pf[3]);
            *(float4 *) (dst + 4) = make_float4(pf[4], pf[5], pf[6], pf[7]);
        }
        __builtin_amdgcn_fence(__ATOMIC_RELEASE, "wavefront");
        __builtin_amdgcn_wave_barrier();
        __builtin_amdgcn_fence(__ATOMIC_ACQUIRE, "wavefront");
#pragma unroll
        for (int hq = 0; hq < 2; hq++) {
            double tot = 0;
#pragma unroll
            for (int c2 = 0; c2 < 8; c2++) tot += (double) prod[hq * 512 + c2 * 64 + lane];
            xa[(hp + hq) * 64 + lane] = (float) tot;
        }
        __builtin_amdgcn_fence(__ATOMIC_RELEASE, "wavefront");
        __builtin_amdgcn_wave_barrier();
        __builtin_amdgcn_fence(__ATOMIC_ACQUIRE, "wavefront");
    }
}

#define MVD_PMAX 4
template <int PRO, int NW, int FMT = MVF_Q4K, int WS = 0, int XB = 4, int RN = 4>
__global__ void __launch_bounds__(NW * 64) matvec_q4k_kernel(mv_args a, int rows_per_wg, attn_args at) {
    constexpr int SB = mvfmt<FMT>::SB, NLOAD = mvfmt<FMT>::NLOAD, TILE = 64 * SB;
    static_assert(WS == 0 || FMT == MVF_Q4K, "the direct layout is written for Q4_K super-blocks");
    auto quantize_block = [&](xblk * dst, const float v[4]) {
        if (FMT == MVF_Q4K) quantize_block_q8k(dst, v, threadIdx.x & 63); else quantize_block_q80((xblk80 *) dst, v, threadIdx.x & 63);
    };
    extern __shared__ __attribute__((aligned(16))) char smem[];
    __shared__ double sh_red[NW];
    const int tid = threadIdx.x, lane = tid & 63, wave = tid >> 6;
#if defined(MV_LOG)
    unsigned mv_log_id = 0;
#endif
    constexpr int nwaves = NW;
    const int nb = (int) (a.K / 256);
    constexpr int STAGE = (WS == 0 || PRO == MV_ATTN) ? TILE : 0;
    xblk * xs = (xblk *) smem;
    char * stage = smem + nb * XBLK_BYTES + wave * STAGE;
    float * part = (float *) (smem + nb * XBLK_BYTES + nwaves * STAGE);

    const bool paired = WS == 0 && a.pair_F > 0;
    const int half_rows = rows_per_wg >> 1;
    const int64_t row0 = paired ? (int64_t) blockIdx.x * half_rows : (int64_t) blockIdx.x * rows_per_wg;
    const int rows = paired ? rows_per_wg : (int) (a.M - row0 < rows_per_wg ? a.M - row0 : rows_per_wg);
    const int nblk = rows * nb;
    const int ntiles = (nblk + 63) >> 6;
    const int nchunks = nblk * (SB / 16);
    const u32x4 * wsrc = (const u32x4 *) (a.w + row0 * a.row_bytes);
    const int tiles_half = paired ? (half_rows * nb) >> 6 : 0x7fffffff;
    const u32x4 * wsrc_r = paired ? (const u32x4 *) (a.w + (a.pair_F + row0) * a.row_bytes) - (int64_t) tiles_half * (NLOAD * 64) : wsrc;

    MV_STAMP(0);
    const int K = (int) a.K;
    float4 xv[XB], aux[XB];
    bool ok[XB];
    auto load_batch = [&](int base) {
#pragma unroll
        for (int j = 0; j < XB; j++) {
            const int e0 = base + j * (NW * 256) + tid * 4;
            ok[j] = e0 < K;
            const int e = ok[j] ? e0 : K - 4;
            xv[j] = *(const float4 *) (a.x + e);
            aux[j] = xv[j];
            if (PRO == MV_RMSNORM) aux[j] = *(const float4 *) (a.alpha + e);
            if (PRO == MV_GATE_SILU) aux[j] = *(const float4 *) (a.x + K + e);
        }
    };
    auto load_batch_tail = [&](int base) {
#pragma unroll
        for (int j = 0; j < XB; j++) {
            const int e0 = base + j * (NW * 256) + tid * 4;
            ok[j] = e0 < K;
            xv[j] = make_float4(0.f, 0.f, 0.f, 0.f); aux[j] = xv[j];
            if (__builtin_amdgcn_readfirstlane(e0 - lane * 4) < K) {
                xv[j] = *(const float4 *) (a.x + e0);
                aux[j] = xv[j];
                if (PRO == MV_RMSNORM) aux[j] = *(const float4 *) (a.alpha + e0);
                if (PRO == MV_GATE_SILU) aux[j] = *(const float4 *) (a.x + K + e0);
            }
        }
    };
    if (PRO != MV_PREQ8K && PRO != MV_ATTN) load_batch(0);
    constexpr int PQ_MAX = 4;
    u32x4 pq[PQ_MAX];
    if (PRO == MV_PREQ8K) {
        const int nchunk = nb * (XBLK_BYTES / 16);
#pragma unroll
        for (int j = 0; j < PQ_MAX; j++) {
            const int i = tid + j * NW * 64;
            pq[j] = ((const u32x4 *) a.x)[i < nchunk ? i : nchunk - 1];
        }
    }
    __builtin_amdgcn_sched_barrier(0);
#if defined(MV_HEAD_EXP) && MV_HEAD_EXP == 1
    __builtin_amdgcn_s_barrier();
#elif defined(MV_HEAD_EXP) && MV_HEAD_EXP == 2
    asm volatile("s_waitcnt vmcnt(0)" ::: "memory");
#endif

    u32x4 r[WS == 0 ? NLOAD : 1];
    u32x4 dh[WS == 1 ? MVD_PMAX : 1], dq[WS == 1 ? MVD_PMAX : 1];
    int t = wave;
    constexpr bool first_is_last = false;
    if (WS == 0 && first_is_last) {
    } else
    if (WS == 0) {
        const bool has_tile = t < ntiles;
#pragma unroll
        for (int i = 0; i < NLOAD; i++) {
            const int g = t * (NLOAD * 64) + i * 64 + lane;
            r[i] = __builtin_nontemporal_load((t >= tiles_half ? wsrc_r : wsrc) + (has_tile ? (g < nchunks ? g : nchunks - 1) : 0));
        }
    } else {
#pragma unroll
        for (int p = 0; p < MVD_PMAX; p++) {
            const int sb = p * (NW * 8) + wave * 8 + (lane >> 3);
            const u32x4 * src = wsrc + (sb < nblk ? sb : nblk - 1) * 9;
            dh[p] = __builtin_nontemporal_load(src);
            dq[p] = __builtin_nontemporal_load(src + 1 + (lane & 7));
        }
    }
    float res_pre[4] = { 0.f, 0.f, 0.f, 0.f };
    if (RN > 0) {
        const float * rp = a.residual ? a.residual : a.y;
#pragma unroll
        for (int k = 0; k < RN; k++) {
            const int rr = (tid >> 4) + k * (NW * 4);
            res_pre[k] = rp[row0 + (rr < (paired ? half_rows : rows) ? rr : 0)];
        }
    }
    __builtin_amdgcn_sched_barrier(0);
    MV_STAMP(1);

    if (PRO == MV_ATTN) {
        float * wbuf = (float *) stage;
        float * xa_all = part + rows_per_wg * nb;
        const int hpw = at.H / NW;
        if (hpw == 4) attn_small_wave<4>(at, wave * 4, lane, wbuf, xa_all + wave * 256, blockIdx.x == 0);
        else          attn_small_wave<2>(at, wave * 2, lane, wbuf, xa_all + wave * 128, blockIdx.x == 0);
        lds_barrier();
        if (wave < nb) {
            float v[4];
#pragma unroll
            for (int k = 0; k < 4; k++) v[k] = xa_all[wave * 256 + lane * 4 + k];
            if (a.x_out != nullptr && blockIdx.x == 0) *(float4 *) (a.x_out + wave * 256 + lane * 4) = make_float4(v[0], v[1], v[2], v[3]);
            quantize_block(xs + wave, v);
        }
    } else if (PRO == MV_PREQ8K) {
        const int nchunk = nb * (XBLK_BYTES / 16);
#pragma unroll
        for (int j = 0; j < PQ_MAX; j++) {
            const int i = tid + j * NW * 64;
            if (i < nchunk) ((u32x4 *) xs)[i] = pq[j];
        }
    } else {
        for (int base = 0; base < K; base += NW * 256 * XB) {
            if (base > 0) load_batch_tail(base);
            float v[XB][4];
#pragma unroll
            for (int j = 0; j < XB; j++) {
                const float z = ok[j] ? 1.f : 0.f;
                v[j][0] = xv[j].x * z; v[j][1] = xv[j].y * z; v[j][2] = xv[j].z * z; v[j][3] = xv[j].w * z;
            }
#if defined(MV_LOG)
            asm volatile("" :: "v"(v[0][0]), "v"(v[XB - 1][3]));
            MV_STAMP(8);
#endif
            if (PRO == MV_RMSNORM) {
                double acc = 0;
#pragma unroll
                for (int j = 0; j < XB; j++)
#pragma unroll
                    for (int k = 0; k < 4; k++) acc += (double) (v[j][k] * v[j][k]);
                acc = wave_allsum_f64(acc);
                if (lane == 0) sh_red[wave] = acc;
                __syncthreads();
                MV_STAMP(9);
                double tot = 0;
#pragma unroll
                for (int w = 0; w < NW; w++) tot += sh_red[w];
                const float mean = (float) (tot / (double) K);
                const float scale = 1.0f / sqrtf(mean + a.eps);
#pragma unroll
                for (int j = 0; j < XB; j++) {
                    const float al[4] = { aux[j].x, aux[j].y, aux[j].z, aux[j].w };
#pragma unroll
                    for (int k = 0; k < 4; k++) v[j][k] = al[k] * (v[j][k] * scale);
                }
            }
            if (PRO == MV_GATE_SILU) {
#pragma unroll
                for (int j = 0; j < XB; j++) {
                    const float rr[4] = { aux[j].x, aux[j].y, aux[j].z, aux[j].w };
#pragma unroll
                    for (int k = 0; k < 4; k++) { const float l = v[j][k]; v[j][k] = (l / (1.0f + expf(-l))) * rr[k]; }
                }
            }
#if defined(MV_LOG)
            asm volatile("" :: "v"(v[0][0]), "v"(v[XB - 1][3]));
            MV_STAMP(10);
#endif
#pragma unroll
            for (int j = 0; j < XB; j++) {
                if (!ok[j]) continue;
                const int b = base / 256 + j * NW + wave;
                if (a.x_out != nullptr && blockIdx.x == 0) *(float4 *) (a.x_out + base + j * (NW * 256) + tid * 4) = make_float4(v[j][0], v[j][1], v[j][2], v[j][3]);
                quantize_block(xs + b, v[j]);
            }
        }
    }
    MV_STAMP(2);
    __syncthreads();
    MV_STAMP(3);

    if (WS == 1) {
#pragma unroll
        for (int p = 0; p < MVD_PMAX; p++) {
            const int sb = p * (NW * 8) + wave * 8 + (lane >> 3);
            if (p * (NW * 8) >= nblk) break;
            const int j8 = lane & 7, g32 = j8 >> 1, hf = j8 & 1;
            const xblk * xb = xs + ((sb < nblk ? sb : nblk - 1) % nb);
            const uint32_t hw[4] = { dh[p].x, dh[p].y, dh[p].z, dh[p].w };
            uint32_t sc[2], mn[2];
            q4k_unpack_scales_w(hw[1], hw[2], hw[3], sc, mn);
            const u32x4 ylo = *(const u32x4 *) (xb->q + 64 * g32 + 16 * hf), yhi = *(const u32x4 *) (xb->q + 64 * g32 + 32 + 16 * hf);
            const uint32_t qw[4] = { dq[p].x, dq[p].y, dq[p].z, dq[p].w }, yl[4] = { ylo.x, ylo.y, ylo.z, ylo.w }, yh[4] = { yhi.x, yhi.y, yhi.z, yhi.w };
            int lo = 0, hi = 0;
#pragma unroll
            for (int k = 0; k < 4; k++) {
                lo = dot4_i8((int) (qw[k] & 0x0F0F0F0Fu), (int) yl[k], lo);
                hi = dot4_i8((int) ((qw[k] >> 4) & 0x0F0F0F0Fu), (int) yh[k], hi);
            }
            const int i0 = 2 * g32, i1 = 2 * g32 + 1;
            const int s0 = (int) ((sc[i0 >> 2] >> (8 * (i0 & 3))) & 0xff), s1 = (int) ((sc[i1 >> 2] >> (8 * (i1 & 3))) & 0xff);
            int isum = __mul24(s0, lo) + __mul24(s1, hi);
            const uint32_t bs2 = *(const uint32_t *) (xb->bsums + 2 * j8);
            const int bs = (int) (int16_t) (bs2 & 0xffff) + (int) (int16_t) (bs2 >> 16);
            int msum = __mul24((int) ((mn[j8 >> 2] >> (8 * (j8 & 3))) & 0xff), bs);
// ... 939 lines not shown

static int env_int(const char * name, int def) { const char * v = getenv(name); return v ? atoi(v) : def; }

void k_matvec(hipStream_t s, const mv_args & a) {
    if (a.wtype == GGML_TYPE_Q4_K || a.wtype == GGML_TYPE_Q8_0 || a.wtype == GGML_TYPE_Q4_0) {
        const int nb = (int) (a.K / 256);
        const int fmt = a.wtype == GGML_TYPE_Q4_K ? MVF_Q4K : a.wtype == GGML_TYPE_Q8_0 ? MVF_Q80 : MVF_Q40;
        const size_t tile_bytes = fmt == MVF_Q80 ? 64 * 272 : 64 * 144;
        static const int force_nw = env_int("MI355X_MV_NW", 0), tpw_min = env_int("MI355X_MV_TPW", 4), grid_min = env_int("MI355X_MV_GRID_MIN", 128);
        const int64_t tiles_total = (a.M * nb + 63) / 64;
        int nw = 4, rows;
        static const int big_tiles = env_int("MI355X_MV_BIG_TILES", 256 * 6), w12_tiles = env_int("MI355X_MV_12W_TILES", 1 << 30);
        if (force_nw ? force_nw > 4 : tiles_total >= big_tiles) {
            nw = force_nw ? force_nw : (tiles_total >= w12_tiles ? 12 : 8);
            rows = (int) ((a.M + 255) / 256);
            while (rows * nb > 4096) rows = (rows + 1) / 2;
        } else {
            int tpw = tpw_min > nb / 4 ? tpw_min : nb / 4;
            rows = (tpw * 64 + nb - 1) / nb;
            if (rows * nb > 4096) rows = 4096 / nb;
            while (rows > 1 && (a.M + rows - 1) / rows < grid_min && (rows / 2) * nb >= 64) rows >>= 1;
        }
        if (a.prologue == MV_ATTN) {
            static const int attn_nw = env_int("MI355X_ATTN_PROLOGUE_NW", 8);
            const int H = a.attn->H;
            GGML_ASSERT(a.K == 1024 && H == 16);
            nw = attn_nw == 4 ? 4 : 8;
            static const int attn_grid_min = env_int("MI355X_ATTN_GRID_MIN", 128);
            int tpw = 4;
            rows = (tpw * 64 + nb - 1) / nb;
            while (rows > 1 && (a.M + rows - 1) / rows < attn_grid_min && (rows / 2) * nb >= 32) rows >>= 1;
        }
        static const int q80_nw = env_int("MI355X_Q80_NW", 8);
        if (fmt == MVF_Q80 && nw > 4 && a.prologue != MV_ATTN) {
            const size_t need8 = (size_t) nb * XBLK_BYTES + 8 * tile_bytes + (size_t) rows * nb * 4;
            if (q80_nw == 8 && need8 <= 158 * 1024) nw = 8;
            else {
                nw = 4;
                rows = (int) ((a.M + 511) / 512);
                while (rows * nb > 4096) rows = (rows + 1) / 2;
            }
        }
        if (a.pair_F > 0) {
            GGML_ASSERT(a.M == 2 * a.pair_F && fmt != MVF_Q80);
            int h = (int) ((a.pair_F + 255) / 256);
            while ((h * nb) % 64 != 0) h++;
            GGML_ASSERT(a.pair_F % h == 0 && 2 * h * nb <= 4096);
            nw = 8; rows = 2 * h;
        }
        if (rows < 1) rows = 1;
        static const int direct_on = env_int("MI355X_MV_DIRECT", 1), direct_passes = env_int("MI355X_MVD_PASSES", 3), direct_max_tiles = env_int("MI355X_MVD_MAX_TILES", 512);
        const bool direct = direct_on && a.pair_F == 0 && fmt == MVF_Q4K && (nw == 4 || (nw == 8 && a.prologue == MV_ATTN)) && tiles_total <= direct_max_tiles && nb <= nw * 8 * MVD_PMAX;
        if (direct) {
            int passes = direct_passes < 1 ? 1 : direct_passes > MVD_PMAX ? MVD_PMAX : direct_passes;
            if (nw == 8 && passes > 1) passes = 1;
            rows = passes * nw * 8 / nb;
            if (rows < 1) { rows = 1; }
            while (rows > 1 && (a.M + rows - 1) / rows < 96) rows = (rows + 1) / 2;
            GGML_ASSERT(rows * nb <= MVD_PMAX * nw * 8);
        }
        const size_t stage_bytes = (!direct || a.prologue == MV_ATTN) ? (size_t) nw * tile_bytes : 0;
        const size_t smem = (size_t) nb * XBLK_BYTES + stage_bytes + (size_t) rows * nb * 4 + (a.prologue == MV_ATTN ? 4096 : 0);
        GGML_ASSERT(smem <= 160 * 1024);
        const int grid = a.pair_F > 0 ? (int) (a.pair_F / (rows / 2)) : (int) ((a.M + rows - 1) / rows);
        GGML_ASSERT(a.prologue != MV_RMSNORM || a.K <= nw * 1024);
        GGML_ASSERT(a.ncols == 1 && a.out_scale == nullptr && (a.prologue <= MV_GATE_SILU || a.prologue == MV_PREQ8K || a.prologue == MV_ATTN));
        void (*kern)(mv_args, int, attn_args) = nullptr;
#define MV_PICKF(NWV, F) (a.prologue == MV_RMSNORM ? matvec_q4k_kernel<MV_RMSNORM, NWV, F> : a.prologue == MV_GATE_SILU ? matvec_q4k_kernel<MV_GATE_SILU, NWV, F> \
                      : a.prologue == MV_ATTN ? matvec_q4k_kernel<MV_ATTN, NWV, F> \
                      : a.prologue == MV_PREQ8K ? matvec_q4k_kernel<MV_PREQ8K, NWV, F> : matvec_q4k_kernel<MV_PLAIN, NWV, F>)
#define MV_PICK(NWV) (fmt == MVF_Q4K ? MV_PICKF(NWV, MVF_Q4K) : fmt == MVF_Q40 ? MV_PICKF(NWV, MVF_Q40) : MV_PICKF(NWV, MVF_Q80))
#define MV_PICKD (a.prologue == MV_RMSNORM ? matvec_q4k_kernel<MV_RMSNORM, 4, MVF_Q4K, 1> : a.prologue == MV_GATE_SILU ? matvec_q4k_kernel<MV_GATE_SILU, 4, MVF_Q4K, 1> \
                  : a.prologue == MV_ATTN ? (nw == 8 ? matvec_q4k_kernel<MV_ATTN, 8, MVF_Q4K, 1> : matvec_q4k_kernel<MV_ATTN, 4, MVF_Q4K, 1>) \
                  : a.prologue == MV_PREQ8K ? matvec_q4k_kernel<MV_PREQ8K, 4, MVF_Q4K, 1> : matvec_q4k_kernel<MV_PLAIN, 4, MVF_Q4K, 1>)
        kern = direct ? MV_PICKD : nw == 12 ? MV_PICK(12) : nw == 8 ? MV_PICK(8) : MV_PICK(4);
        static const int lean_on = env_int("MI355X_MV_LEAN", 1);
        if (lean_on && !direct && nw == 8 && fmt == MVF_Q4K && a.prologue == MV_RMSNORM && a.K <= 8 * 512 && !a.residual && !a.res_embed.table)
            kern = matvec_q4k_kernel<MV_RMSNORM, 8, MVF_Q4K, 0, 2, 0>;
        if (lean_on && !direct && fmt == MVF_Q4K && a.prologue == MV_PLAIN && a.pair_F == 0 && a.residual && rows <= nw * 4 && (nw == 8 || nw == 4))
            kern = nw == 8 ? matvec_q4k_kernel<MV_PLAIN, 8, MVF_Q4K, 0, 4, 1> : matvec_q4k_kernel<MV_PLAIN, 4, MVF_Q4K, 0, 4, 1>;
        static const int one_round = env_int("MI355X_MV_ONE_ROUND", 1);
        if (lean_on && one_round && !direct && fmt == MVF_Q4K && a.prologue == MV_PLAIN && a.pair_F == 0 && a.residual && rows <= nw * 4 && nw == 8 && a.K > 8 * 1024 && a.K <= 8 * 1536)
            kern = matvec_q4k_kernel<MV_PLAIN, 8, MVF_Q4K, 0, 6, 1>;
        if (smem > 64 * 1024) {
            static std::map<const void *, size_t> granted;
            size_t & g = granted[(const void *) kern];
            if (g < smem) { HIP_CHECK(hipFuncSetAttribute((const void *) kern, hipFuncAttributeMaxDynamicSharedMemorySize, (int) smem)); g = smem; }
        }
        const int threads = nw * 64;
        attn_args at;
        memset(&at, 0, sizeof(at));
        if (a.prologue == MV_ATTN) at = *a.attn;
        if (g_mv_profile && g_mv_profile->used < g_mv_profile->capacity) {
            mv_profile::rec & r = g_mv_profile->recs[g_mv_profile->used++];
            r.bytes = a.M * a.row_bytes;
            r.variant = direct ? 1 : 0;
            hipExtLaunchKernelGGL(kern, dim3(grid), dim3(threads), smem, s, r.start, r.stop, 0, a, rows, at);
            return;
        }
        kern<<<grid, threads, smem, s>>>(a, rows, at);
        return;
    }
    GGML_ASSERT(a.ncols >= 1 && a.ncols <= MV_MAX_COLS);
    static const int no_reg = env_int("MI355X_MV_NOREG", 0);
    if (a.wtype == GGML_TYPE_F32 && !no_reg && (a.K == 512 || a.K == 1024 || a.K == 2048) && a.row_bytes % 16 == 0 && ((uintptr_t) a.w % 16) == 0) {
        static const int two_min = env_int("MI355X_MVF_TWO_MIN", 4 * 2 * 256);
        const bool two = a.K <= 1024 && a.M >= two_min;
        const int grid = (int) ((a.M + (two ? 8 : 4) - 1) / (two ? 8 : 4));
        if (a.K == 512)       { if (two) matvec_f32_reg_kernel<2, 2><<<grid, 256, 0, s>>>(a); else matvec_f32_reg_kernel<2, 1><<<grid, 256, 0, s>>>(a); }
        else if (a.K == 1024) { if (two) matvec_f32_reg_kernel<4, 2><<<grid, 256, 0, s>>>(a); else matvec_f32_reg_kernel<4, 1><<<grid, 256, 0, s>>>(a); }
        else                  matvec_f32_reg_kernel<8, 1><<<grid, 256, 0, s>>>(a);
        return;
    }
    int rows_per_wave = a.K <= 1024 ? 4 : 2;
    while (rows_per_wave > 1 && (a.M + 4 * rows_per_wave - 1) / (4 * rows_per_wave) < 256) rows_per_wave >>= 1;
    const int grid = (int) ((a.M + 4 * rows_per_wave - 1) / (4 * rows_per_wave));
    const size_t smem = (size_t) a.K * 4 * (size_t) a.ncols;
    switch (a.wtype) {
        case GGML_TYPE_F32:  matvec_f_kernel<GGML_TYPE_F32><<<grid, 256, smem, s>>>(a, rows_per_wave); break;
        case GGML_TYPE_F16:  matvec_f_kernel<GGML_TYPE_F16><<<grid, 256, smem, s>>>(a, rows_per_wave); break;
        case GGML_TYPE_BF16: matvec_f_kernel<GGML_TYPE_BF16><<<grid, 256, smem, s>>>(a, rows_per_wave); break;
        default: GGML_ABORT("k_matvec: unsupported weight type");
    }
}

#define ATTN_BODY_LOG
#include "hip_attn_body.h"

template <bool SPLIT, int NWA>
__global__ void __launch_bounds__(NWA * 64) __attribute__((amdgpu_waves_per_eu(2)))
attn_decode_kernel(attn_args a_in, attn_split_ws w) {
    extern __shared__ __attribute__((aligned(16))) char smem[];
    const int S = SPLIT ? w.S : 1;
    attn_decode_body<SPLIT, NWA, AT_PLAIN>(a_in, w, smem, SPLIT ? (int) blockIdx.x / S : (int) blockIdx.x, SPLIT ? (int) blockIdx.x % S : 0, (int) blockIdx.y);
}

static bool attn_use_split(const attn_args & a) { return a.T == 1 && a.n_groups <= 1 && a.D == 128 && a.C >= ATTN_SPLIT_MIN_C; }
static int attn_split_nw() { static const int v = env_int("MI355X_ATTN_SPLIT_NW", ATTN_SPLIT_NW_DEFAULT); return v == 8 ? 8 : 4; }
static int attn_split_slots() { static const int v = env_int("MI355X_ATTN_SLOTS", attn_split_nw() == 8 ? 192 : ATTN_SPLIT_SLOTS); return v < 64 ? 64 : v > 32 * attn_split_nw() ? 32 * attn_split_nw() : v; }
size_t k_attn_decode_ws_size(const attn_args & a) {
    if (!attn_use_split(a)) return 0;
    const size_t S = (size_t) (a.C + attn_split_slots() - 1) / attn_split_slots();
    return 256 + (((size_t) a.H * 4 + 255) & ~(size_t) 255) + (size_t) a.H * a.C * 8 + (size_t) a.H * S * a.D * 16;
}
static size_t attn_smem_bytes(const attn_args & a, bool split, bool wide) {
    const int Tg = a.n_groups > 1 ? ATTN_MAX_T : a.T;
    return (size_t) a.C * 4 + (size_t) Tg * a.D * 4 * 3 + (size_t) (split ? attn_split_nw() : wide ? ATTN_NW_WIDE : ATTN_NW_BASE) * 64 * 8 * 8 + 16 + (size_t) Tg * a.C * 4 + (size_t) env_int("MI355X_ATTN_LDS_PAD", 0);
}
bool k_attn_split_resident(const attn_args & a, int usable_cus) {
    if (!attn_use_split(a)) return false;
    if (env_int("MI355X_ATTN_SPLIT_FORCE", 0)) return true;
    const int nw = attn_split_nw();
    const size_t smem = attn_smem_bytes(a, true, false);
    const void * fn = nw == 8 ? (const void *) attn_decode_kernel<true, ATTN_NW_WIDE> : (const void *) attn_decode_kernel<true, ATTN_NW_BASE>;
    if (smem > 64 * 1024 && hipFuncSetAttribute(fn, hipFuncAttributeMaxDynamicSharedMemorySize, (int) smem) != hipSuccess) return false;
    int per_cu = 0;
    if (hipOccupancyMaxActiveBlocksPerMultiprocessor(&per_cu, fn, nw * 64, smem) != hipSuccess) return false;
    const long long grid = (long long) a.H * ((a.C + attn_split_slots() - 1) / attn_split_slots());
    const bool ok = (long long) per_cu * usable_cus >= grid;
    if (env_int("MI355X_CHAIN_VERBOSE", 0)) fprintf(stderr, "split attention: grid %lld, %d per CU x %d CUs -> %s\n", grid, per_cu, usable_cus, ok ? "split" : "one workgroup per head");
    return ok;
}
__global__ void __launch_bounds__(512) attn_ring64_kernel(attn_args a) {
    extern __shared__ __attribute__((aligned(16))) char smem[];
    attn_ring64_body<AT_PLAIN>(a, smem, (int) blockIdx.x);
}
// ... 94 lines not shown
attn_blocks_kernel(attn_blocks_args ba, attn_split_ws w) {
    extern __shared__ __attribute__((aligned(16))) char smem[];
    const attn_block_job & jb = ba.job[blockIdx.z];
    const int groups = (jb.T + ATTN_MAX_T - 1) / ATTN_MAX_T;
    if ((int) blockIdx.x >= groups) return;
    attn_args a = ba.a;
    a.q = jb.q; a.k = jb.k; a.v = jb.v;
    a.kcache = jb.kcache; a.vcache = jb.vcache;
    a.mask = jb.mask; a.rot = jb.rot; a.index = jb.index; a.out = jb.out;
    a.T = jb.T; a.n_groups = groups; a.write_only = ba.write_only; a.row_split = 0;
    attn_decode_body<false, NWA, AT_PLAIN>(a, w, smem, (int) blockIdx.y, 0, (int) blockIdx.x);
}
void k_attn_blocks(hipStream_t s, const attn_blocks_args & ba, unsigned * err) {
    const attn_args & a = ba.a;
    GGML_ASSERT(ba.n_jobs >= 1 && ba.n_jobs <= ATTN_BLOCKS_MAX);
    GGML_ASSERT(a.D % 8 == 0 && 64 % (a.D / 8) == 0 && ATTN_MAX_T * a.D <= 2 * ATTN_NW_BASE * 64);
    int max_groups = 1;
    for (int j = 0; j < ba.n_jobs; j++) {
        GGML_ASSERT(ba.job[j].T >= 1 && ba.job[j].T <= 64);
        const int g = (ba.job[j].T + ATTN_MAX_T - 1) / ATTN_MAX_T;
        if (g > max_groups) max_groups = g;
    }
    static const int wide_on = env_int("MI355X_ATTN_WIDE", 1);
    const bool wide = wide_on && a.D <= 64 && a.C >= 128;
    attn_args sized = a; sized.n_groups = 2;
    const size_t smem = attn_smem_bytes(sized, false, wide);
    GGML_ASSERT(smem <= 160 * 1024);
    if (smem > 64 * 1024) {
        static size_t granted[2] = { 0, 0 };
        if (granted[wide] < smem) {
            HIP_CHECK(hipFuncSetAttribute(wide ? (const void *) attn_blocks_kernel<ATTN_NW_WIDE> : (const void *) attn_blocks_kernel<ATTN_NW_BASE>,
                                          hipFuncAttributeMaxDynamicSharedMemorySize, (int) smem));
            granted[wide] = smem;
        }
    }
    static const int single_max = env_int("MI355X_ATTN_SINGLE_MAX", ATTN_SINGLE_MAX), big_min = env_int("MI355X_ATTN_BIG_MIN", ATTN_SPLIT_BIG_MIN);
    const attn_split_ws w = { nullptr, nullptr, nullptr, 1, err, ATTN_SPLIT_SLOTS, single_max, big_min };
    const dim3 grid((unsigned) max_groups, (unsigned) a.H, (unsigned) ba.n_jobs);
    if (wide) attn_blocks_kernel<ATTN_NW_WIDE><<<grid, ATTN_NW_WIDE * 64, smem, s>>>(ba, w);
    else      attn_blocks_kernel<ATTN_NW_BASE><<<grid, ATTN_NW_BASE * 64, smem, s>>>(ba, w);
}

__global__ void __launch_bounds__(256) copy_rows_kernel(copy_rows_args a) {
    const int r = (int) blockIdx.y;
    const int64_t i = (int64_t) blockIdx.x * 256 + threadIdx.x;
    if (r >= a.rows || i >= a.n) return;
    a.dst[(int64_t) r * a.n + i] = a.src[r][i];
}
void k_copy_rows(hipStream_t s, const copy_rows_args & a) {
    GGML_ASSERT(a.rows >= 1 && a.rows <= COPY_ROWS_MAX && a.n >= 1);
    const dim3 grid((unsigned) ((a.n + 255) / 256), (unsigned) a.rows);
    copy_rows_kernel<<<grid, 256, 0, s>>>(a);
}

__global__ void __launch_bounds__(256) ring_copy_kernel(ring_copy_args a) {
    const int bpr = a.blocks_per_run;
    const int run = (int) blockIdx.x / bpr, part = (int) blockIdx.x % bpr;
    const int j = run / a.H, h = run % a.H;
    const ring_copy_job & jb = a.job[j];
    const uint4 * __restrict__ src = (const uint4 *) (jb.src + (int64_t) h * jb.src_hs);
    uint4 * __restrict__ dst = (uint4 *) (jb.dst + (int64_t) h * jb.dst_hs);
    const int64_t nvec = a.run_bytes >> 4, per = (nvec + bpr - 1) / bpr;
    const int64_t begin = (int64_t) part * per, end = begin + per < nvec ? begin + per : nvec;
    int64_t i = begin + threadIdx.x;
    for (; i + 3 * 256 < end; i += 4 * 256) {
        const uint4 v0 = src[i], v1 = src[i + 256], v2 = src[i + 512], v3 = src[i + 768];
        dst[i] = v0; dst[i + 256] = v1; dst[i + 512] = v2; dst[i + 768] = v3;
    }
    for (; i < end; i += 256) dst[i] = src[i];
}
void k_ring_copy(hipStream_t s, const ring_copy_args & in, int usable_cus) {
    GGML_ASSERT(in.n_jobs >= 1 && in.n_jobs <= RING_COPY_MAX && in.H >= 1 && in.run_bytes >= 16 && in.run_bytes % 16 == 0);
    ring_copy_args a = in;
    const int64_t runs = (int64_t) a.n_jobs * a.H, target = 8 * (int64_t) (usable_cus > 0 ? usable_cus : 256);
    int64_t bpr = (target + runs - 1) / runs;
    const int64_t most = (a.run_bytes + 16383) / 16384;
    if (bpr > most) bpr = most;
    if (bpr < 1) bpr = 1;
    a.blocks_per_run = (int) bpr;
    ring_copy_kernel<<<(unsigned) (runs * bpr), 256, 0, s>>>(a);
}

#define FOLD_NW 8
#define FOLD_GRID 256
#define FOLD_PMAX 4
struct fold_ws { unsigned long long * gbuf; unsigned long long * arrive; unsigned * err; };
#if defined(MV_LOG)
#define FD_STAMP(i) do { if (blockIdx.x == 0 && threadIdx.x == 0) { unsigned long long t_; asm volatile("s_memrealtime %0\n\ts_waitcnt lgkmcnt(0)" : "=s"(t_) :: "memory"); g_fold_log[fd_id][i] = t_; } } while (0)
__device__ unsigned long long g_fold_log[4096][8];
__device__ unsigned g_fold_launch;
extern "C" __attribute__((visibility("default"))) int mi355x_fold_log_read(unsigned long long * out, int max_records) {
    unsigned n = 0;
    if (hipMemcpyFromSymbol(&n, HIP_SYMBOL(g_fold_launch), 4) != hipSuccess) return -1;
    const int m = (int) (n < 4096u ? n : 4096u) < max_records ? (int) (n < 4096u ? n : 4096u) : max_records;
    if (hipMemcpyFromSymbol(out, HIP_SYMBOL(g_fold_log), (size_t) m * 8 * 8) != hipSuccess) return -1;
    const unsigned z = 0; (void) hipMemcpyToSymbol(HIP_SYMBOL(g_fold_launch), &z, 4);
    return (int) n;
}
#else
#define FD_STAMP(i) do {} while (0)
#endif

static int fold_split_S(const attn_args & at) { return FOLD_GRID / at.H; }
static bool fold_use_split(const attn_args & at) {
    if (!attn_use_split(at)) return false;
    static const int big_min = env_int("MI355X_ATTN_BIG_MIN", ATTN_SPLIT_BIG_MIN);
    const int S = fold_split_S(at), slots = env_int("MI355X_FOLD_SLOTS", 192);
    return (int64_t) S * slots >= (at.C < big_min ? at.C : big_min) && (int64_t) 2 * S * slots >= at.C;
}
template <bool SPLIT, int NJ>
__global__ void __launch_bounds__(FOLD_NW * 64) inproj_attn_kernel(mv_args a, attn_args at, attn_split_ws w, fold_ws f, attn_gqkv gq, int seg_rows, int64_t seg_stride) {
    constexpr int NW = FOLD_NW, NLOAD = 9, SB = 144, TILE = 64 * SB;
    extern __shared__ __attribute__((aligned(16))) char smem[];
    __shared__ double sh_red[NW];
    const int tid = threadIdx.x, lane = tid & 63, wave = tid >> 6;
    const int b = blockIdx.x, H = at.H, S = (int) gridDim.x / H;
    const int h = b % H, part_i = b / H;
    const int blk = h * S + part_i;
#if defined(MV_LOG)
    __shared__ unsigned fd_id_s;
    if (b == 0 && tid == 0) fd_id_s = atomicAdd(&g_fold_launch, 1u) & 4095u;
    __syncthreads();
    const unsigned fd_id = b == 0 ? fd_id_s : 0u;
#endif
    FD_STAMP(0);
    const unsigned tag = (unsigned) (__hip_atomic_load(f.arrive, __ATOMIC_RELAXED, __HIP_MEMORY_SCOPE_AGENT) / (unsigned long long) FOLD_GRID) + 1u;
    const int nb = (int) (a.K / 256), K = (int) a.K;
    const int rows = 3 * seg_rows, nblk = rows * nb, ntiles = nblk >> 6, tiles_seg = (seg_rows * nb) >> 6;
    xblk * xs = (xblk *) smem;
    char * stage = smem + nb * XBLK_BYTES + wave * TILE;
    float * part = (float *) (smem + nb * XBLK_BYTES + NW * TILE);
    auto tile_src = [&](int t) {
        const int sg = t / tiles_seg;
        return (const u32x4 *) (a.w + ((int64_t) sg * seg_stride + (int64_t) blk * seg_rows) * a.row_bytes) + (int64_t) (t - sg * tiles_seg) * (NLOAD * 64);
    };
    float4 xv[NJ], aux[NJ];
    bool ok[NJ];
#pragma unroll
    for (int j = 0; j < NJ; j++) {
        const int e0 = j * (NW * 256) + tid * 4;
        ok[j] = e0 < K;
        const int e = ok[j] ? e0 : K - 4;
        xv[j] = *(const float4 *) (a.x + e);
        aux[j] = *(const float4 *) (a.alpha + e);
    }
    __builtin_amdgcn_sched_barrier(0);
#if defined(MV_HEAD_EXP) && MV_HEAD_EXP == 1
    __builtin_amdgcn_s_barrier();
#elif defined(MV_HEAD_EXP) && MV_HEAD_EXP == 2
    asm volatile("s_waitcnt vmcnt(0)" ::: "memory");
#endif
    u32x4 r[NLOAD];
    int t = wave;
    {
        const bool has_tile = t < ntiles;
        const u32x4 * src = tile_src(has_tile ? t : 0);
#pragma unroll
        for (int i = 0; i < NLOAD; i++) r[i] = __builtin_nontemporal_load(src + (has_tile ? i * 64 + lane : 0));
    }
    __builtin_amdgcn_sched_barrier(0);
    {
        float v[NJ][4];
#pragma unroll
        for (int j = 0; j < NJ; j++) {
            const float z = ok[j] ? 1.f : 0.f;
            v[j][0] = xv[j].x * z; v[j][1] = xv[j].y * z; v[j][2] = xv[j].z * z; v[j][3] = xv[j].w * z;
        }
        double acc = 0;
#pragma unroll
        for (int j = 0; j < NJ; j++)
#pragma unroll
            for (int k = 0; k < 4; k++) acc += (double) (v[j][k] * v[j][k]);
        acc = wave_allsum_f64(acc);
        if (lane == 0) sh_red[wave] = acc;
        __syncthreads();
        double tot = 0;
#pragma unroll
        for (int w_ = 0; w_ < NW; w_++) tot += sh_red[w_];
        const float mean = (float) (tot / (double) K);
        const float scale = 1.0f / sqrtf(mean + a.eps);
#pragma unroll
        for (int j = 0; j < NJ; j++) {
            const float al[4] = { aux[j].x, aux[j].y, aux[j].z, aux[j].w };
#pragma unroll
            for (int k = 0; k < 4; k++) v[j][k] = al[k] * (v[j][k] * scale);
        }
#pragma unroll
        for (int j = 0; j < NJ; j++) {
            if (!ok[j]) continue;
            const int bq = j * NW + wave;
            if (a.x_out != nullptr && b == 0) *(float4 *) (a.x_out + j * (NW * 256) + tid * 4) = make_float4(v[j][0], v[j][1], v[j][2], v[j][3]);
            quantize_block_q8k(xs + bq, v[j], lane);
        }
    }
    __syncthreads();
    FD_STAMP(1);
    for (; t < ntiles; t += NW) {
#pragma unroll
        for (int i = 0; i < NLOAD; i++) ((u32x4 *) stage)[i * 64 + lane] = r[i];
        {
            const int tn = t + NW < ntiles ? t + NW : ntiles - 1;
            const u32x4 * src = tile_src(tn);
#pragma unroll
            for (int i = 0; i < NLOAD; i++) r[i] = __builtin_nontemporal_load(src + i * 64 + lane);
        }
        __builtin_amdgcn_fence(__ATOMIC_RELEASE, "wavefront");
        __builtin_amdgcn_wave_barrier();
        __builtin_amdgcn_fence(__ATOMIC_ACQUIRE, "wavefront");
        const int bi = t * 64 + lane;
        const xblk * xb = xs + (bi % nb);
        part[bi] = q4k_q8k_block_dot((const block_q4_K *) (stage + lane * SB), xb->q, xb->bsums, xb->d);
        __builtin_amdgcn_wave_barrier();
    }
    __syncthreads();
    FD_STAMP(2);
    for (int rr = tid >> 4; rr < rows; rr += NW * 4) {
        float sum = 0.f;
        for (int j = tid & 15; j < nb; j += 16) sum += part[rr * nb + j];
        sum = row16_allsum_f32(sum);
        if ((tid & 15) == 0) {
            const int sg = rr / seg_rows;
            const int64_t row = (int64_t) sg * seg_stride + (int64_t) blk * seg_rows + (rr - sg * seg_rows);
            a.y[row] = sum;
            __hip_atomic_store(f.gbuf + row, ((unsigned long long) tag << 32) | (unsigned long long) __float_as_uint(sum), __ATOMIC_RELAXED, __HIP_MEMORY_SCOPE_AGENT);
        }
    }
    __syncthreads();
    FD_STAMP(3);
    attn_decode_body<SPLIT, NW, AT_GQKV>(at, w, smem, h, part_i, 0, tag, gq);
    FD_STAMP(4);
    if (tid == 0) { asm volatile("" :: "v"(tag) : "memory"); (void) __hip_atomic_fetch_add(f.arrive, 1ull, __ATOMIC_RELAXED, __HIP_MEMORY_SCOPE_AGENT); }
    FD_STAMP(5);
}

typedef void (*fold_kernel_t)(mv_args, attn_args, attn_split_ws, fold_ws, attn_gqkv, int, int64_t);
static fold_kernel_t fold_kernel_fn(bool split, int K) {
    const int nj = (K + FOLD_NW * 256 - 1) / (FOLD_NW * 256);
    GGML_ASSERT(nj >= 1 && nj <= 2);
    return split ? (nj == 1 ? inproj_attn_kernel<true, 1> : inproj_attn_kernel<true, 2>) : (nj == 1 ? inproj_attn_kernel<false, 1> : inproj_attn_kernel<false, 2>);
}
static const void * fold_kernel(bool split, int K) { return (const void *) fold_kernel_fn(split, K); }
static size_t inproj_attn_smem(const mv_args & a, const attn_args & at, int seg_rows) {
    const size_t attn = (size_t) at.C * 4 + (size_t) at.T * at.D * 4 * 3 + (size_t) FOLD_NW * 64 * 8 * 8 + 16 + (size_t) at.T * at.C * 4;
    const size_t mv = (size_t) (a.K / 256) * XBLK_BYTES + (size_t) FOLD_NW * 64 * 144 + (size_t) 3 * seg_rows * (a.K / 256) * 4;
    return ((attn > mv ? attn : mv) + 15) & ~(size_t) 15;
}
bool k_inproj_attn_supported(const mv_args & a, const attn_args & at, int usable_cus) {
    static const int on = env_int("MI355X_INPROJ_ATTN", 1);
    if (!on) return false;
    if (a.wtype != GGML_TYPE_Q4_K || a.ncols != 1 || a.prologue != MV_RMSNORM || a.pair_F || a.out_scale || a.out_act || a.ticket || a.res_embed.table || a.residual ||
        a.argmax_out[0] || a.argmax_out[1]) return false;
    if (a.K % 256 != 0 || a.K > 4096 || a.K < 256 || a.row_bytes != (a.K / 256) * 144 || ((uintptr_t) a.w & 15)) return false;
    if (at.C <= 32 || at.T != 1 || at.n_groups > 1 || at.H < 1 || FOLD_GRID % at.H != 0 || at.D != 128) return false;
    const int64_t HD = (int64_t) at.H * at.D;
    if (a.M != 3 * HD || HD % FOLD_GRID != 0) return false;
    const int seg_rows = (int) (HD / FOLD_GRID), nb = (int) (a.K / 256);
    if ((seg_rows * nb) % 64 != 0 || 3 * seg_rows * nb > 4096 || (at.D % seg_rows) != 0 || (seg_rows & 1)) return false;
    if (at.q != a.y || at.k != a.y + HD || at.v != a.y + 2 * HD || at.q_hs != at.D || at.k_hs != at.D || at.v_hs != at.D) return false;
    if (attn_use_split(at) && !fold_use_split(at)) return false;
    const size_t smem = inproj_attn_smem(a, at, seg_rows);
    if (smem > 160 * 1024) return false;
    const void * fn = fold_kernel(fold_use_split(at), (int) a.K);
    if (smem > 64 * 1024 && hipFuncSetAttribute(fn, hipFuncAttributeMaxDynamicSharedMemorySize, (int) smem) != hipSuccess) return false;
    if (env_int("MI355X_FOLD_FORCE", 0)) return true;
    int per_cu = 0;
    if (hipOccupancyMaxActiveBlocksPerMultiprocessor(&per_cu, fn, FOLD_NW * 64, smem) != hipSuccess) return false;
    return (long long) per_cu * usable_cus >= FOLD_GRID;
}
size_t k_inproj_attn_ws_size(const mv_args & a, const attn_args & at) {
    size_t n = 256 + (size_t) a.M * 8;
    if (fold_use_split(at)) n += (((size_t) at.H * 4 + 255) & ~(size_t) 255) + (size_t) at.H * at.C * 8 + (size_t) at.H * fold_split_S(at) * at.D * 16;
    return n;
}
void k_inproj_attn(hipStream_t s, const mv_args & a, const attn_args & at, void * ws, unsigned * err) {
    static const int single_max = env_int("MI355X_ATTN_SINGLE_MAX", ATTN_SINGLE_MAX), big_min = env_int("MI355X_ATTN_BIG_MIN", ATTN_SPLIT_BIG_MIN);
    char * p = (char *) ws;
    fold_ws f = { (unsigned long long *) (p + 256), (unsigned long long *) p, err };
    p += 256 + (size_t) a.M * 8;
    const bool split = fold_use_split(at);
    attn_split_ws w = { nullptr, nullptr, nullptr, 1, err, ATTN_SPLIT_SLOTS, single_max, big_min };
    if (split) {
        w.slots = env_int("MI355X_FOLD_SLOTS", 192);
        w.S = fold_split_S(at);
        w.seq = (unsigned *) p; p += ((size_t) at.H * 4 + 255) & ~(size_t) 255;
        w.gscores = (unsigned long long *) p; p += (size_t) at.H * at.C * 8;
        w.gpart = (unsigned long long *) p;
    }
    const int64_t HD = (int64_t) at.H * at.D;
    const int seg_rows = (int) (HD / FOLD_GRID);
    const attn_gqkv gq = { f.gbuf, 0, HD, 2 * HD, err };
    const size_t smem = inproj_attn_smem(a, at, seg_rows);
    const fold_kernel_t fold_fn = fold_kernel_fn(split, (int) a.K);
    if (g_mv_profile && g_mv_profile->used < g_mv_profile->capacity) {
        mv_profile::rec & r = g_mv_profile->recs[g_mv_profile->used++];
        r.bytes = a.M * a.row_bytes;
        r.variant = 2;
        hipExtLaunchKernelGGL(fold_fn, dim3(FOLD_GRID), dim3(FOLD_NW * 64), smem, s, r.start, r.stop, 0, a, at, w, f, gq, seg_rows, HD);
        return;
    }
    fold_fn<<<FOLD_GRID, FOLD_NW * 64, smem, s>>>(a, at, w, f, gq, seg_rows, HD);
}

__global__ void __launch_bounds__(256) cross_attn_kernel(xattn_args a) {
    extern __shared__ float xsm[];
    __shared__ float sh_f[4];
    __shared__ double sh_d[4];
    const int h = blockIdx.x, tid = threadIdx.x, lane = tid & 63, wave = tid >> 6;
    const int D = a.D, Tc = a.Tc;
    float * qs = xsm, * sc = xsm + D;
    for (int d = tid; d < D; d += 256) qs[d] = a.q[(int64_t) h * D + d];
    __syncthreads();
    const char * kh = a.k + (int64_t) h * a.k_nb2, * vh = a.v + (int64_t) h * a.v_nb2;
    for (int t0 = wave * 4; t0 < Tc; t0 += 16) {
        double acc[4] = { 0, 0, 0, 0 };
        for (int d = lane; d < D; d += 64) {
            float kv[4];
#pragma unroll
            for (int u = 0; u < 4; u++) kv[u] = *(const float *) (kh + (int64_t) (t0 + u < Tc ? t0 + u : Tc - 1) * a.k_nb1 + (int64_t) d * 4);
#pragma unroll
            for (int u = 0; u < 4; u++) acc[u] += (double) (kv[u] * qs[d]);
        }
#pragma unroll
        for (int u = 0; u < 4; u++) {
            const double r = wave_allsum_f64(acc[u]);
            if (lane == 0 && t0 + u < Tc) sc[t0 + u] = (float) r;
        }
    }
    __syncthreads();
    float mx = -INFINITY;
    for (int t = tid; t < Tc; t += 256) mx = fmaxf(mx, sc[t] * a.scale);
    mx = wave_allmax_f32(mx);
    if (lane == 0) sh_f[wave] = mx;
    __syncthreads();
    mx = fmaxf(fmaxf(sh_f[0], sh_f[1]), fmaxf(sh_f[2], sh_f[3]));
    double sum = 0;
    for (int t = tid; t < Tc; t += 256) { const float e = expf(sc[t] * a.scale - mx); sc[t] = e; sum += (double) e; }
    sum = wave_allsum_f64(sum);
    if (lane == 0) sh_d[wave] = sum;
    __syncthreads();
    const float inv = (float) (1.0 / (sh_d[0] + sh_d[1] + sh_d[2] + sh_d[3]));
    for (int t = tid; t < Tc; t += 256) sc[t] *= inv;
    __syncthreads();
    {
        const int G = 256 / D > 0 ? 256 / D : 1, grp = tid / D, d = tid - grp * D;
        double acc = 0;
        if (grp < G) {
            const int per = (Tc + G - 1) / G, tb = grp * per, te = tb + per < Tc ? tb + per : Tc;
            for (int t = tb; t < te; t += 8) {
                float vv[8];
#pragma unroll
                for (int u = 0; u < 8; u++) vv[u] = *(const float *) (vh + (int64_t) (t + u < te ? t + u : te - 1) * a.v_nb1 + (int64_t) d * 4);
#pragma unroll
                for (int u = 0; u < 8; u++) if (t + u < te) acc += (double) (vv[u] * sc[t + u]);
            }
        }
        double * part = (double *) (xsm + ((D + Tc + 1) & ~1));
        if (grp < G) part[grp * D + d] = acc;
        __syncthreads();
        if (tid < D) {
            double tot = 0;
            for (int gi = 0; gi < G; gi++) tot += part[gi * D + tid];
            a.out[(int64_t) h * D + tid] = (float) tot;
        }
    }
}
void k_cross_attn(hipStream_t s, const xattn_args & a) {
    GGML_ASSERT(a.D <= 256);
    const size_t smem = (size_t) ((a.D + a.Tc + 1) & ~1) * 4 + (size_t) (256 / a.D > 0 ? 256 / a.D : 1) * a.D * 8;
    GGML_ASSERT(smem <= 64 * 1024);
    cross_attn_kernel<<<a.H, 256, smem, s>>>(a);
}

template <int TYPE, int NMAX>
__global__ void __launch_bounds__(64) embed_sum_kernel(embed_sum_args a) {
    const int64_t i = (int64_t) blockIdx.x * blockDim.x + threadIdx.x;
    if (i >= a.K) return;
    const int b = (int) blockIdx.y;
    int64_t r[NMAX];
    float sc[NMAX], v[NMAX];
#pragma unroll
    for (int t = 0; t < NMAX; t++) {
        const embed_src & e = a.src[t < a.n ? t : 0];
        r[t] = e.index[b];
// ... 354 lines not shown
```

Measured before the change: 445.4 frames/s.

## Pair attention heads in fused in-proj kernel and pre-quantize output for out-projection

In the fused in-projection+attention kernel, even heads now compute attention for two heads at once in the short-context quick path, while odd-head blocks skip their attention work. The paired block then quantizes its 256-element output into a q8_K block and publishes it with a generation tag. A new MV_PLAIN_PREQ matvec variant reads these pre-quantized blocks and skips its own activation quantization when every tag matches, falling back to normal quantization otherwise. This is meant to remove quantization work and latency from the out-projection. The cost is extra shared memory, more register pressure in the paired blocks and uneven work across blocks. A probe API and a stats counter are added for validation.

```diff
diff --git a/include/ggml-backend.h b/include/ggml-backend.h
--- a/include/ggml-backend.h
+++ b/include/ggml-backend.h
@@ -102,6 +102,7 @@
     int64_t generic_attention_nodes_in_last_plan;
     int64_t ring_copy_launches_in_last_plan;
     int64_t ring_copy_jobs_in_last_plan;
+    int64_t attention_preq_planned;
 };
 GGML_API void ggml_backend_mi355x_get_stats(ggml_backend_t backend, struct ggml_mi355x_stats * stats);
 struct ggml_mi355x_kernel_profile {
@@ -116,6 +117,7 @@
     int64_t chain_bytes;
     int64_t chain_phases;
 };
+GGML_API int64_t ggml_backend_mi355x_attn_preq_probe(ggml_backend_t backend, void * out, size_t max_bytes);
 GGML_API void ggml_backend_mi355x_get_kernel_profile(ggml_backend_t backend, struct ggml_mi355x_kernel_profile * out);
 GGML_API void ggml_backend_mi355x_set_flags(ggml_backend_t backend, int flags);
 GGML_API void ggml_backend_mi355x_set_capture(ggml_backend_t backend, int enabled);
diff --git a/moshi.cpp_amd/__init__.py b/moshi.cpp_amd/__init__.py
--- a/moshi.cpp_amd/__init__.py
+++ b/moshi.cpp_amd/__init__.py
@@ -49,7 +49,7 @@
                                          "fused_nodes_in_last_plan", "nodes_in_last_plan", "uploads_batched", "chained_matvecs_in_last_plan",
                                          "attention_folds_planned", "chain_step_programs_in_last_plan", "vq_levels_chained_in_last_plan",
                                          "attn_block_launches_in_last_plan", "attn_block_jobs_in_last_plan", "generic_attention_nodes_in_last_plan",
-                                         "ring_copy_launches_in_last_plan", "ring_copy_jobs_in_last_plan")]
+                                         "ring_copy_launches_in_last_plan", "ring_copy_jobs_in_last_plan", "attention_preq_planned")]
 
 
 class KernelProfile(C.Structure):
@@ -122,7 +122,7 @@
     "ggml_backend_tensor_set": (None, [TP, P, Z, Z]), "ggml_backend_tensor_get": (None, [TP, P, Z, Z]),
     "ggml_backend_tensor_memset": (None, [TP, C.c_uint8, Z, Z]), "ggml_backend_tensor_copy": (None, [TP, TP]),
     "ggml_backend_graph_compute": (I, [P, P]), "ggml_backend_supports_op": (B, [P, TP]),
-    "ggml_backend_mi355x_get_stats": (None, [P, C.POINTER(Stats)]), "ggml_backend_mi355x_set_flags": (None, [P, I]), "ggml_backend_mi355x_set_capture": (None, [P, I]),
+    "ggml_backend_mi355x_get_stats": (None, [P, C.POINTER(Stats)]), "ggml_backend_mi355x_attn_preq_probe": (L, [P, P, Z]), "ggml_backend_mi355x_set_flags": (None, [P, I]), "ggml_backend_mi355x_set_capture": (None, [P, I]),
     "ggml_backend_mi355x_get_stream": (P, [P]),
     "ggml_backend_mi355x_make_current": (None, [P]),
     "ggml_backend_mi355x_init_stream": (P, [P]),
diff --git a/moshi.cpp_amd/csrc/hip_attn_body.h b/moshi.cpp_amd/csrc/hip_attn_body.h
--- a/moshi.cpp_amd/csrc/hip_attn_body.h
+++ b/moshi.cpp_amd/csrc/hip_attn_body.h
@@ -1,5 +1,6 @@
 #pragma once
 #include "hip_device.h"
+#include "hip_mv_device.h"
 
 #define ATTN_NW_BASE 4
 #define ATTN_NW_WIDE 8
@@ -18,13 +19,20 @@
 #else
 #define AT_STAMP(i) do {} while (0)
 #endif
+#ifndef ATTN_QUICK
+#define ATTN_QUICK 1
+#endif
+#define ATTN_QUICK_ON (ATTN_QUICK != 0)
+#define ATTN_PAIR_SMEM_EXTRA(C) ((size_t) 128 * 4 * 3 + (size_t) (C) * 4 + 16 + (size_t) 8 * 64 * 8 * 8 + 256 * 4)
 #ifndef ATTN_V_EARLY
 #define ATTN_V_EARLY 0
 #endif
 #define AT_PLAIN 0
 #define AT_GQKV  2
 #define AT_GOUT  4
+#define AT_PAIR  8
 struct attn_gqkv { const unsigned long long * in; int64_t qoff, koff, voff; unsigned * err; };
+struct attn_pair { xblk * blocks; int follow; };
 struct attn_gout { unsigned long long * out; unsigned tag; int64_t ts;
 #if defined(CH_LOG)
                    unsigned long long * log;
@@ -37,8 +45,9 @@
 #endif
 template <bool SPLIT, int NWA, int MODE>
 __device__ __forceinline__ void attn_decode_body(const attn_args & a_in, const attn_split_ws & w, char * smem, const int h, const int s_idx, const int group_y,
-                                                 const unsigned gtag = 0u, const attn_gqkv gq = attn_gqkv(), const attn_gout go = attn_gout()) {
-    constexpr bool GQKV = (MODE & AT_GQKV) != 0, GOUT = (MODE & AT_GOUT) != 0;
+                                                 const unsigned gtag = 0u, const attn_gqkv gq = attn_gqkv(), const attn_gout go = attn_gout(), const attn_pair pr = attn_pair()) {
+    constexpr bool GQKV = (MODE & AT_GQKV) != 0, GOUT = (MODE & AT_GOUT) != 0, PAIR = (MODE & AT_PAIR) != 0;
+    static_assert(!PAIR || (GQKV && !GOUT && NWA == 8), "paired heads: the merged launch's short-ring form");
     constexpr int ATTN_NW = NWA, ATTN_THREADS = NWA * 64;
 #if defined(MV_LOG)
     unsigned at_log_id = 0;
@@ -56,17 +65,21 @@
     }
     constexpr int NB = SPLIT ? (NWA == 8 ? 8 : 12) : ATTN_NPRE;
     constexpr int NPRE = ATTN_NPRE;
-    const int D = SPLIT ? 128 : a.D, C = a.C, T = SPLIT ? 1 : a.T;
+    const int D = (SPLIT || PAIR) ? 128 : a.D, C = a.C, T = (SPLIT || PAIR) ? 1 : a.T;
+    const int NE = PAIR ? 2 * D : T * D;
     const int S = SPLIT ? w.S : 1;
     int SLOTS = SPLIT ? w.slots : ATTN_SPLIT_SLOTS;
     int c_base = s_idx * SLOTS;
     const int tid = threadIdx.x, lane = tid & 63, wave = tid >> 6;
     float * sc   = (float *) smem;
     float * qf   = sc + C;
-    float * knew = qf + T * D;
-    float * vnew = knew + T * D;
-    double * red = (double *) (smem + (((size_t) (C + 3 * T * D) * 4 + 15) & ~(size_t) 15));
+    float * knew = qf + NE;
+    float * vnew = knew + NE;
+    double * red = (double *) (smem + (((size_t) (C + 3 * NE) * 4 + 15) & ~(size_t) 15));
     float * msk = (float *) (red + ATTN_NW * (64 / (D / 8)) * D);
+    float * sc2 = msk + T * C;
+    double * red2 = (double *) (smem + (((((size_t) (C + 3 * NE) * 4 + 15) & ~(size_t) 15) + (size_t) ATTN_NW * 64 * 8 * 8 + (size_t) 2 * T * C * 4 + 15) & ~(size_t) 15));
+    float * xo = (float *) (red2 + ATTN_NW * 64 * 8);
     __shared__ float sh_f[ATTN_NW];
     __shared__ double sh_d[ATTN_NW];
     __shared__ int sh_i[ATTN_NW];
@@ -139,11 +152,11 @@
 #pragma unroll
     for (int u = 0; u < 2; u++) {
         const int e = tid + u * ATTN_THREADS;
-        const int ee = e < T * D ? e : 0;
-        const int t = ee / D, j = ee - t * D;
-        const float * q = a.q + (int64_t) t * a.q_ts + (int64_t) h * a.q_hs;
-        const float * k = a.k + (int64_t) t * a.k_ts + (int64_t) h * a.k_hs;
-        const float * v = a.v + (int64_t) t * a.v_ts + (int64_t) h * a.v_hs;
+        const int ee = e < NE ? e : 0;
+        const int r = ee / D, j = ee - r * D, t = PAIR ? 0 : r, hq = PAIR ? h + r : h;
+        const float * q = a.q + (int64_t) t * a.q_ts + (int64_t) hq * a.q_hs;
+        const float * k = a.k + (int64_t) t * a.k_ts + (int64_t) hq * a.k_hs;
+        const float * v = a.v + (int64_t) t * a.v_ts + (int64_t) hq * a.v_hs;
         if (!GQKV) in_v[u] = v[j];
         if (a.rot) {
             const int p = j < half ? j : j - half;
@@ -169,14 +182,24 @@
         kpre[pi] = *(const uint4 *) (kc + (int64_t) cc * a.k_nb1 + dl * 2);
         if (pi < ATTN_NPRE) vpre[pi] = *(const uint4 *) (vc + (int64_t) cc * a.v_nb1 + dl * 2);
     }
+    uint4 kpre2[PAIR ? NPRE : 1], vpre2[PAIR ? NPRE : 1];
+    if (PAIR) {
+#pragma unroll
+        for (int pi = 0; pi < NPRE; pi++) {
+            const int c = c_base + wave * SPW + pi * ATTN_NW * SPW + sub;
+            const int cc = c < C ? c : C - 1;
+            kpre2[pi] = *(const uint4 *) (kc + a.k_nb2 + (int64_t) cc * a.k_nb1 + dl * 2);
+            vpre2[pi] = *(const uint4 *) (vc + a.v_nb2 + (int64_t) cc * a.v_nb1 + dl * 2);
+        }
+    }
     if (GQKV) {
 #pragma unroll
         for (int u = 0; u < 2; u++) {
             const int e = tid + u * ATTN_THREADS;
             in_q0[u] = in_q1[u] = in_k0[u] = in_k1[u] = in_v[u] = 0.f;
-            if (e < T * D) {
-                const int t = e / D, j = e - t * D, p = j < half ? j : j - half;
-                const int64_t eq = (int64_t) t * a.q_ts + (int64_t) h * a.q_hs, ek = (int64_t) t * a.k_ts + (int64_t) h * a.k_hs, ev = (int64_t) t * a.v_ts + (int64_t) h * a.v_hs;
+            if (e < NE) {
+                const int r = e / D, j = e - r * D, p = j < half ? j : j - half, t = PAIR ? 0 : r, hq = PAIR ? h + r : h;
+                const int64_t eq = (int64_t) t * a.q_ts + (int64_t) hq * a.q_hs, ek = (int64_t) t * a.k_ts + (int64_t) hq * a.k_hs, ev = (int64_t) t * a.v_ts + (int64_t) hq * a.v_hs;
                 const unsigned long long * gp[5] = { gq.in + gq.qoff + eq + (a.rot ? 2 * p : j), gq.in + gq.qoff + eq + (a.rot ? 2 * p + 1 : j),
                                                      gq.in + gq.koff + ek + (a.rot ? 2 * p : j), gq.in + gq.koff + ek + (a.rot ? 2 * p + 1 : j), gq.in + gq.voff + ev + j };
                 unsigned long long g[5];
@@ -218,8 +241,8 @@
 #pragma unroll
     for (int u = 0; u < 2; u++) {
         const int e = tid + u * ATTN_THREADS;
-        if (e < T * D) {
-            const int t = e / D, j = e - t * D;
+        if (e < NE) {
+            const int r = e / D, j = e - r * D, t = PAIR ? 0 : r;
             float qo, ko;
             if (a.rot) {
                 if (j < half) { qo = in_q0[u] * in_c[u] - in_q1[u] * in_s[u]; ko = in_k0[u] * in_c[u] - in_k1[u] * in_s[u]; }
@@ -230,9 +253,9 @@
             knew[e] = bf2f(kb);
             vnew[e] = bf2f(vb);
             const int slot = slot_t[t < ATTN_MAX_T ? t : 0];
-            if (s_idx == 0 && (SPLIT || !a.row_split || group_y == 0) && slot >= 0 && slot < C) {
-                ((uint16_t *) (kc + (int64_t) slot * a.k_nb1))[j] = kb;
-                ((uint16_t *) (vc + (int64_t) slot * a.v_nb1))[j] = vb;
+            if (s_idx == 0 && (SPLIT || !a.row_split || group_y == 0) && slot >= 0 && slot < C && !pr.follow) {
+                ((uint16_t *) (kc + (PAIR ? (int64_t) r * a.k_nb2 : 0) + (int64_t) slot * a.k_nb1))[j] = kb;
+                ((uint16_t *) (vc + (PAIR ? (int64_t) r * a.v_nb2 : 0) + (int64_t) slot * a.v_nb1))[j] = vb;
             }
         }
     }
@@ -242,6 +265,8 @@
     AT_STAMP(2);
     const int P = SPLIT && n_end > w.single_max ? (n_end + SLOTS - 1) / SLOTS : 1;
     const bool multi = SPLIT && P > 1;
+    const bool quick = ATTN_QUICK_ON && !multi && T == 1 && n_end <= 128 && n_end <= NPRE * ATTN_NW * SPW;
+    if (pr.follow && quick) return;
     const int c_lo = multi ? c_base : 0, c_hi = multi ? min(n_end, c_base + SLOTS) : n_end;
     const int c_last = c_hi > 0 ? c_hi - 1 : 0;
     auto pack_row = [&](const float * src) {
@@ -258,6 +283,7 @@
     for (int pi = 0; pi < NPRE; pi++) {
         const int f = fresh_of(c_base + wave * SPW + pi * ATTN_NW * SPW + sub);
         if (f >= 0) { kpre[pi] = pack_row(knew + f * D + dl); if (pi < ATTN_NPRE) vpre[pi] = pack_row(vnew + f * D + dl); }
+        if (PAIR && f >= 0) { kpre2[pi] = pack_row(knew + D + dl); vpre2[pi] = pack_row(vnew + D + dl); }
     }
     AT_STAMP(8);
 
@@ -317,6 +343,27 @@
             const int c0 = c_lo + wave * SPW + pi * ATTN_NW * SPW;
             if (c0 < c_hi) score_pass(c0, kpre[pi]);
         }
+        if (PAIR && quick) {
+            float qv2[8];
+#pragma unroll
+            for (int i = 0; i < 8; i++) qv2[i] = qf[D + dl + i];
+#pragma unroll
+            for (int pi = 0; pi < NPRE; pi++) {
+                const int c0 = c_lo + wave * SPW + pi * ATTN_NW * SPW, c = c0 + sub;
+                if (c0 < c_hi) {
+                    const float m = c < c_hi ? mask[c] : -INFINITY;
+                    const uint32_t kw[4] = { kpre2[pi].x, kpre2[pi].y, kpre2[pi].z, kpre2[pi].w };
+                    double acc = 0;
+#pragma unroll
+                    for (int i = 0; i < 4; i++) {
+                        acc += (double) (bf2f((uint16_t) (kw[i] & 0xffff)) * qv2[2 * i]);
+                        acc += (double) (bf2f((uint16_t) (kw[i] >> 16)) * qv2[2 * i + 1]);
+                    }
+                    acc = group_allsum_f64(acc, LPS);
+                    if (c < c_hi && (lane % LPS) == 0) sc2[c] = m > -INFINITY ? (float) acc * a.scale + m : -INFINITY;
+                }
+            }
+        }
         for (int cb = cb_first; cb < c_hi; cb += NB * ATTN_NW * SPW) {
             if (!SPLIT || cb != cb_first) request_k_batch(cb);
 #pragma unroll
@@ -337,10 +384,7 @@
             }
         }
         AT_STAMP(10);
-#ifndef ATTN_QUICK
-#define ATTN_QUICK 1
-#endif
-        if (ATTN_QUICK && !multi && T == 1 && n_end <= 128 && n_end <= NPRE * ATTN_NW * SPW) {
+        if (quick) {
             __syncthreads();
             AT_STAMP(3);
             const float s0 = lane < n_end ? sc[lane] : -INFINITY, s1 = lane + 64 < n_end ? sc[lane + 64] : -INFINITY;
@@ -348,6 +392,14 @@
             const float e0 = s0 > -INFINITY ? expf(s0 - qmax) : 0.f, e1 = s1 > -INFINITY ? expf(s1 - qmax) : 0.f;
             const double qsum = wave_allsum_f64((double) e0 + (double) e1);
             const float qinv = (float) (1.0 / qsum);
+            float qmax2 = 0.f, qinv2 = 0.f;
+            if (PAIR) {
+                const float t0 = lane < n_end ? sc2[lane] : -INFINITY, t1 = lane + 64 < n_end ? sc2[lane + 64] : -INFINITY;
+                qmax2 = wave_allmax_f32(fmaxf(t0, t1));
+                const float f0 = t0 > -INFINITY ? expf(t0 - qmax2) : 0.f, f1 = t1 > -INFINITY ? expf(t1 - qmax2) : 0.f;
+                const double qsum2 = wave_allsum_f64((double) f0 + (double) f1);
+                qinv2 = (float) (1.0 / qsum2);
+            }
             AT_STAMP(4);
             double q8[8];
 #pragma unroll
@@ -367,6 +419,28 @@
                     }
                 }
             }
+            if (PAIR) {
+                double p8[8];
+#pragma unroll
+                for (int i = 0; i < 8; i++) p8[i] = 0;
+#pragma unroll
+                for (int pi = 0; pi < NPRE; pi++) {
+                    const int c0 = c_lo + wave * SPW + pi * ATTN_NW * SPW, c = c0 + sub;
+                    if (c0 < c_hi) {
+                        const float sv = c < c_hi ? sc2[c] : -INFINITY;
+                        const float e = sv > -INFINITY ? expf(sv - qmax2) : 0.f;
+                        const float pq = c < c_hi ? bf2f(f2bf(e * qinv2)) : 0.f;
+                        const uint32_t vw[4] = { vpre2[pi].x, vpre2[pi].y, vpre2[pi].z, vpre2[pi].w };
+#pragma unroll
+                        for (int i = 0; i < 4; i++) {
+                            p8[2 * i]     += (double) (bf2f((uint16_t) (vw[i] & 0xffff)) * pq);
+                            p8[2 * i + 1] += (double) (bf2f((uint16_t) (vw[i] >> 16)) * pq);
+                        }
+                    }
+                }
+#pragma unroll
+                for (int i = 0; i < 8; i++) red2[(wave * SPW + sub) * D + dl + i] = p8[i];
+            }
             AT_STAMP(5);
 #pragma unroll
             for (int i = 0; i < 8; i++) red[(wave * SPW + sub) * D + dl + i] = q8[i];
@@ -377,6 +451,12 @@
 #pragma unroll
                 for (int g = 0; g < 8; g++) if (g < SPW) tw += red[(wave * SPW + g) * D + j];
                 red[(wave * SPW) * D + j] = tw;
+                if (PAIR) {
+                    double tw2 = 0;
+#pragma unroll
+                    for (int g = 0; g < 8; g++) if (g < SPW) tw2 += red2[(wave * SPW + g) * D + j];
+                    red2[(wave * SPW) * D + j] = tw2;
+                }
             }
             __syncthreads();
             for (int j = tid; j < D; j += ATTN_THREADS) {
@@ -384,7 +464,26 @@
 #pragma unroll
                 for (int w = 0; w < ATTN_NW; w++) tot += red[(w * SPW) * D + j];
                 a.out[(int64_t) t * a.out_ts + (int64_t) h * D + j] = (float) tot;
+                if (PAIR) xo[j] = (float) tot;
                 if (GOUT) __hip_atomic_store(go.out + (int64_t) t * go.ts + (int64_t) h * D + j, ((unsigned long long) go.tag << 32) | (unsigned long long) __float_as_uint((float) tot), __ATOMIC_RELAXED, __HIP_MEMORY_SCOPE_AGENT);
+            }
+            if (PAIR) {
+                if (tid >= D && tid < 2 * D) {
+                    const int j = tid - D;
+                    double tot = 0;
+#pragma unroll
+                    for (int w = 0; w < ATTN_NW; w++) tot += red2[(w * SPW) * D + j];
+                    a.out[(int64_t) t * a.out_ts + (int64_t) (h + 1) * D + j] = (float) tot;
+                    xo[D + j] = (float) tot;
+                }
+                __syncthreads();
+                if (wave == 0) {
+                    xblk * blk = pr.blocks + (h >> 1);
+                    const float4 x4 = *(const float4 *) (xo + lane * 4);
+                    const float v[4] = { x4.x, x4.y, x4.z, x4.w };
+                    quantize_block_q8k(blk, v, lane);
+                    if (lane == 0) __hip_atomic_store((unsigned *) &blk->pad[0], gtag, __ATOMIC_RELAXED, __HIP_MEMORY_SCOPE_AGENT);
+                }
             }
             continue;
         }
diff --git a/moshi.cpp_amd/csrc/hip_backend.hip b/moshi.cpp_amd/csrc/hip_backend.hip
--- a/moshi.cpp_amd/csrc/hip_backend.hip
+++ b/moshi.cpp_amd/csrc/hip_backend.hip
@@ -51,6 +51,7 @@
     uint64_t orphan_clock = 0;
     volatile unsigned * err_host = nullptr;
     unsigned * err_dev = nullptr;
+    void * preq_probe = nullptr; int64_t preq_probe_K = 0;
     char * readback = nullptr;
     struct async_get { void * dst; size_t size; int slot; uint64_t seq; };
     char * aget_pinned = nullptr;
@@ -1958,6 +1959,9 @@
             }
             p->n_fused += 2;
         }
+        struct attn_preq_t { const ggml_tensor * node; int64_t K; const void * blocks; const unsigned long long * arrive; };
+        std::unordered_map<const void *, attn_preq_t> attn_preq;
+        const bool attn_preq_on = !(getenv("MI355X_ATTN_PREQ") != nullptr && atoi(getenv("MI355X_ATTN_PREQ")) == 0);
         std::unordered_map<const void *, float *> paired_gate;
         size_t paired_consumed = 0;
         static const bool no_pair = getenv("MI355X_PAIRED_GATE") != nullptr && atoi(getenv("MI355X_PAIRED_GATE")) == 0;
@@ -2037,7 +2041,21 @@
                     const size_t wn = k_inproj_attn_ws_size(a, at);
                     void * ws = em.ws(wn);
                     HIP_CHECK(hipMemsetAsync(ws, 0, wn, c->stream));
-                    at_pos[ag.emit_pos].insert(at_pos[ag.emit_pos].begin(), [=](hipStream_t s) { k_inproj_attn(s, am, aa, ws, err); });
+                    void * pair_blocks = nullptr;
+                    if (attn_preq_on && k_inproj_attn_pairable(at) && at.out_ts == (int64_t) at.H * at.D) {
+                        const size_t bn = (size_t) (at.H / 2) * MV_XBLK_BYTES;
+                        pair_blocks = em.ws(bn);
+                        HIP_CHECK(hipMemsetAsync(pair_blocks, 0, bn, c->stream));
+                        attn_preq[(const void *) at.out] = { g->nodes[ag.emit_pos], (int64_t) at.H * at.D, pair_blocks, (const unsigned long long *) ws };
+                    }
+                    at_pos[ag.emit_pos].insert(at_pos[ag.emit_pos].begin(), [=](hipStream_t s) { k_inproj_attn(s, am, aa, ws, err, pair_blocks); });
+                    if (pair_blocks && getenv("MI355X_ATTN_PREQ_PROBE") != nullptr && atoi(getenv("MI355X_ATTN_PREQ_PROBE")) != 0) {
+                        const int64_t K = (int64_t) at.H * at.D;
+                        void * rec = em.ws(k_attn_preq_probe_size(K));
+                        const float * xo = at.out;
+                        at_pos[ag.emit_pos].insert(at_pos[ag.emit_pos].begin() + 1, [=](hipStream_t s) { k_attn_preq_probe(s, xo, K, pair_blocks, rec); });
+                        c->preq_probe = rec; c->preq_probe_K = K;
+                    }
                     ag.emit_pos = -1;
                     p->n_fused += 1; p->n_attn_folded++; c->stats.attention_folds_planned++;
                     merged = true;
@@ -2077,6 +2095,12 @@
                         }
                     }
                 }
+            }
+            if (a.prologue == MV_PLAIN && a.wtype == GGML_TYPE_Q4_K && a.ncols == 1 && a.pair_F == 0 && attn_preq.count((const void *) a.x)) {
+                const attn_preq_t & pb = attn_preq[(const void *) a.x];
+                const ggml_tensor * xn = g->nodes[i]->src[1];
+                while (xn && xn != pb.node && (xn->op == GGML_OP_VIEW || xn->op == GGML_OP_RESHAPE || xn->op == GGML_OP_PERMUTE || xn->op == GGML_OP_TRANSPOSE)) xn = xn->src[0];
+                if (xn == pb.node && a.K == pb.K && a.x_cs >= 0) { a.preq = pb.blocks; a.preq_arrive = pb.arrive; c->stats.attention_preq_planned++; }
             }
             if (a.prologue == MV_GATE_SILU && is_qblock((enum ggml_type) a.wtype) && a.K > 4096 && paired_gate.count((const void *) a.x)) {
                 const float * gbuf = paired_gate[(const void *) a.x];
@@ -2504,6 +2528,13 @@
     return (hip_ctx *) b->context;
 }
 extern "C" void ggml_backend_mi355x_get_stats(ggml_backend_t b, struct ggml_mi355x_stats * stats) { *stats = ctx_of(b)->stats; }
+extern "C" int64_t ggml_backend_mi355x_attn_preq_probe(ggml_backend_t b, void * out, size_t max_bytes) {
+    hip_ctx * c = ctx_of(b);
+    if (c->preq_probe == nullptr || out == nullptr || max_bytes < k_attn_preq_probe_size(c->preq_probe_K)) return 0;
+    HIP_CHECK(hipStreamSynchronize(c->stream));
+    HIP_CHECK(hipMemcpy(out, c->preq_probe, k_attn_preq_probe_size(c->preq_probe_K), hipMemcpyDeviceToHost));
+    return c->preq_probe_K;
+}
 extern "C" void ggml_backend_mi355x_set_capture(ggml_backend_t b, int enabled) {
     if (b && b->iface.get_name == hip_backend_name) ((hip_ctx *) b->context)->no_capture = !enabled;
 }
diff --git a/moshi.cpp_amd/csrc/hip_common.h b/moshi.cpp_amd/csrc/hip_common.h
--- a/moshi.cpp_amd/csrc/hip_common.h
+++ b/moshi.cpp_amd/csrc/hip_common.h
@@ -63,7 +63,7 @@
 struct upload_desc { char * dst; uint32_t offset; uint32_t size; };
 void k_scatter_uploads(hipStream_t s, const upload_desc * descs, const char * blob, int n);
 
-enum mv_prologue { MV_PLAIN = 0, MV_RMSNORM = 1, MV_GATE_SILU = 2, MV_LAYERNORM = 3, MV_GELU = 4, MV_PREQ8K = 5, MV_ATTN = 6 };
+enum mv_prologue { MV_PLAIN = 0, MV_RMSNORM = 1, MV_GATE_SILU = 2, MV_LAYERNORM = 3, MV_GELU = 4, MV_PREQ8K = 5, MV_ATTN = 6, MV_PLAIN_PREQ = 7  };
 struct attn_args;
 struct embed_src { const char * table; int64_t row_bytes; int64_t n_rows; int type; const int32_t * index; const float * scale; };
 #define MV_MAX_COLS 4
@@ -89,6 +89,8 @@
     unsigned *  ticket;
     const attn_args * attn;
     int64_t     pair_F;
+    const void * preq;
+    const unsigned long long * preq_arrive;
     int         special;
     const struct lowrank_embed_args * lr;
     const struct sample_args * smp;
@@ -157,7 +159,10 @@
 
 bool   k_inproj_attn_supported(const mv_args & a, const attn_args & at, int usable_cus);
 size_t k_inproj_attn_ws_size(const mv_args & a, const attn_args & at);
-void   k_inproj_attn(hipStream_t s, const mv_args & a, const attn_args & at, void * ws, unsigned * err);
+void   k_inproj_attn(hipStream_t s, const mv_args & a, const attn_args & at, void * ws, unsigned * err, void * pair_blocks = nullptr);
+bool   k_inproj_attn_pairable(const attn_args & at);
+size_t k_attn_preq_probe_size(int64_t K);
+void   k_attn_preq_probe(hipStream_t s, const float * x, int64_t K, const void * blocks, void * out);
 
 struct xattn_args { const float * q; const char * k; const char * v; int64_t k_nb1, k_nb2, v_nb1, v_nb2; int H, D, Tc; float scale; float * out; };
 void k_cross_attn(hipStream_t s, const xattn_args & a);
diff --git a/moshi.cpp_amd/csrc/hip_kernels_fused.hip b/moshi.cpp_amd/csrc/hip_kernels_fused.hip
--- a/moshi.cpp_amd/csrc/hip_kernels_fused.hip
+++ b/moshi.cpp_amd/csrc/hip_kernels_fused.hip
@@ -220,6 +220,7 @@
     }
 }
 
+#define FOLD_GRID 256
 #define MVD_PMAX 4
 template <int PRO, int NW, int FMT = MVF_Q4K, int WS = 0, int XB = 4, int RN = 4>
 __global__ void __launch_bounds__(NW * 64) matvec_q4k_kernel(mv_args a, int rows_per_wg, attn_args at) {
@@ -293,6 +294,17 @@
             pq[j] = ((const u32x4 *) a.x)[i < nchunk ? i : nchunk - 1];
         }
     }
+    unsigned pq_tag = 0u; unsigned long long pq_arrive = 0ull;
+    if (PRO == MV_PLAIN_PREQ) {
+        const int nchunk = nb * (XBLK_BYTES / 16);
+#pragma unroll
+        for (int j = 0; j < PQ_MAX; j++) {
+            const int i = tid + j * NW * 64;
+            pq[j] = ((const u32x4 *) a.preq)[i < nchunk ? i : nchunk - 1];
+        }
+        pq_tag = ((const unsigned *) a.preq)[(lane < nb ? lane : nb - 1) * (XBLK_BYTES / 4) + (int) (offsetof(xblk, pad) / 4)];
+        pq_arrive = *a.preq_arrive;
+    }
     __builtin_amdgcn_sched_barrier(0);
 #if defined(MV_HEAD_EXP) && MV_HEAD_EXP == 1
     __builtin_amdgcn_s_barrier();
@@ -334,6 +346,22 @@
     __builtin_amdgcn_sched_barrier(0);
     MV_STAMP(1);
 
+    bool preq_taken = false;
+    if (PRO == MV_PLAIN_PREQ) {
+        preq_taken = __all(pq_tag == (unsigned) (pq_arrive / (unsigned long long) FOLD_GRID)) != 0;
+        if (preq_taken) {
+            const int nchunk = nb * (XBLK_BYTES / 16);
+#pragma unroll
+            for (int j = 0; j < PQ_MAX; j++) {
+                const int i = tid + j * NW * 64;
+                if (i < nchunk) ((u32x4 *) xs)[i] = pq[j];
+            }
+            if (a.x_out != nullptr && blockIdx.x == 0) {
+#pragma unroll
+                for (int j = 0; j < XB; j++) if (ok[j]) *(float4 *) (a.x_out + j * (NW * 256) + tid * 4) = xv[j];
+            }
+        }
+    }
     if (PRO == MV_ATTN) {
         float * wbuf = (float *) stage;
         float * xa_all = part + rows_per_wg * nb;
@@ -355,7 +383,7 @@
             const int i = tid + j * NW * 64;
             if (i < nchunk) ((u32x4 *) xs)[i] = pq[j];
         }
-    } else {
+    } else if (!preq_taken) {
         for (int base = 0; base < K; base += NW * 256 * XB) {
             if (base > 0) load_batch_tail(base);
             float v[XB][4];
@@ -1461,6 +1489,10 @@
         static const int one_round = env_int("MI355X_MV_ONE_ROUND", 1);
         if (lean_on && one_round && !direct && fmt == MVF_Q4K && a.prologue == MV_PLAIN && a.pair_F == 0 && a.residual && rows <= nw * 4 && nw == 8 && a.K > 8 * 1024 && a.K <= 8 * 1536)
             kern = matvec_q4k_kernel<MV_PLAIN, 8, MVF_Q4K, 0, 6, 1>;
+        if (a.preq != nullptr && a.preq_arrive != nullptr && lean_on && !direct && fmt == MVF_Q4K && a.prologue == MV_PLAIN && a.pair_F == 0 && a.residual && rows <= nw * 4 && (nw == 8 || nw == 4) &&
+            a.K <= nw * 1024 && nb <= 64 && nb * (XBLK_BYTES / 16) <= 4 * nw * 64) {
+            kern = nw == 8 ? matvec_q4k_kernel<MV_PLAIN_PREQ, 8, MVF_Q4K, 0, 4, 1> : matvec_q4k_kernel<MV_PLAIN_PREQ, 4, MVF_Q4K, 0, 4, 1>;
+        }
         if (smem > 64 * 1024) {
             static std::map<const void *, size_t> granted;
             size_t & g = granted[(const void *) kern];
@@ -1721,7 +1753,6 @@
 }
 
 #define FOLD_NW 8
-#define FOLD_GRID 256
 #define FOLD_PMAX 4
 struct fold_ws { unsigned long long * gbuf; unsigned long long * arrive; unsigned * err; };
 #if defined(MV_LOG)
@@ -1748,7 +1779,7 @@
     return (int64_t) S * slots >= (at.C < big_min ? at.C : big_min) && (int64_t) 2 * S * slots >= at.C;
 }
 template <bool SPLIT, int NJ>
-__global__ void __launch_bounds__(FOLD_NW * 64) inproj_attn_kernel(mv_args a, attn_args at, attn_split_ws w, fold_ws f, attn_gqkv gq, int seg_rows, int64_t seg_stride) {
+__global__ void __launch_bounds__(FOLD_NW * 64) inproj_attn_kernel(mv_args a, attn_args at, attn_split_ws w, fold_ws f, attn_gqkv gq, int seg_rows, int64_t seg_stride, xblk * pair_blocks) {
     constexpr int NW = FOLD_NW, NLOAD = 9, SB = 144, TILE = 64 * SB;
     extern __shared__ __attribute__((aligned(16))) char smem[];
     __shared__ double sh_red[NW];
@@ -1866,21 +1897,27 @@
     }
     __syncthreads();
     FD_STAMP(3);
-    attn_decode_body<SPLIT, NW, AT_GQKV>(at, w, smem, h, part_i, 0, tag, gq);
+    if (pair_blocks != nullptr && part_i == 0 && !(h & 1)) attn_decode_body<SPLIT, NW, AT_GQKV | AT_PAIR>(at, w, smem, h, part_i, 0, tag, gq, attn_gout(), attn_pair { pair_blocks, 0 });
+    else attn_decode_body<SPLIT, NW, AT_GQKV>(at, w, smem, h, part_i, 0, tag, gq, attn_gout(), attn_pair { nullptr, pair_blocks != nullptr && part_i == 0 && (h & 1) });
     FD_STAMP(4);
     if (tid == 0) { asm volatile("" :: "v"(tag) : "memory"); (void) __hip_atomic_fetch_add(f.arrive, 1ull, __ATOMIC_RELAXED, __HIP_MEMORY_SCOPE_AGENT); }
     FD_STAMP(5);
 }
 
-typedef void (*fold_kernel_t)(mv_args, attn_args, attn_split_ws, fold_ws, attn_gqkv, int, int64_t);
+typedef void (*fold_kernel_t)(mv_args, attn_args, attn_split_ws, fold_ws, attn_gqkv, int, int64_t, xblk *);
 static fold_kernel_t fold_kernel_fn(bool split, int K) {
     const int nj = (K + FOLD_NW * 256 - 1) / (FOLD_NW * 256);
     GGML_ASSERT(nj >= 1 && nj <= 2);
     return split ? (nj == 1 ? inproj_attn_kernel<true, 1> : inproj_attn_kernel<true, 2>) : (nj == 1 ? inproj_attn_kernel<false, 1> : inproj_attn_kernel<false, 2>);
 }
 static const void * fold_kernel(bool split, int K) { return (const void *) fold_kernel_fn(split, K); }
+static bool fold_pairable(const attn_args & at) {
+    return at.H % 2 == 0 && at.D == 128 && at.T == 1 && (at.C & 3) == 0 && (((uintptr_t) at.mask) & 15) == 0 && at.C / 4 <= 3 * FOLD_NW * 64;
+}
+bool k_inproj_attn_pairable(const attn_args & at) { return fold_pairable(at); }
 static size_t inproj_attn_smem(const mv_args & a, const attn_args & at, int seg_rows) {
-    const size_t attn = (size_t) at.C * 4 + (size_t) at.T * at.D * 4 * 3 + (size_t) FOLD_NW * 64 * 8 * 8 + 16 + (size_t) at.T * at.C * 4;
+    size_t attn = (size_t) at.C * 4 + (size_t) at.T * at.D * 4 * 3 + (size_t) FOLD_NW * 64 * 8 * 8 + 16 + (size_t) at.T * at.C * 4;
+    if (fold_pairable(at)) attn += ATTN_PAIR_SMEM_EXTRA(at.C);
     const size_t mv = (size_t) (a.K / 256) * XBLK_BYTES + (size_t) FOLD_NW * 64 * 144 + (size_t) 3 * seg_rows * (a.K / 256) * 4;
     return ((attn > mv ? attn : mv) + 15) & ~(size_t) 15;
 }
@@ -1911,7 +1948,8 @@
     if (fold_use_split(at)) n += (((size_t) at.H * 4 + 255) & ~(size_t) 255) + (size_t) at.H * at.C * 8 + (size_t) at.H * fold_split_S(at) * at.D * 16;
     return n;
 }
-void k_inproj_attn(hipStream_t s, const mv_args & a, const attn_args & at, void * ws, unsigned * err) {
+void k_inproj_attn(hipStream_t s, const mv_args & a, const attn_args & at, void * ws, unsigned * err, void * pair_blocks) {
+    GGML_ASSERT(pair_blocks == nullptr || fold_pairable(at));
     static const int single_max = env_int("MI355X_ATTN_SINGLE_MAX", ATTN_SINGLE_MAX), big_min = env_int("MI355X_ATTN_BIG_MIN", ATTN_SPLIT_BIG_MIN);
     char * p = (char *) ws;
     fold_ws f = { (unsigned long long *) (p + 256), (unsigned long long *) p, err };
@@ -1934,10 +1972,26 @@
         mv_profile::rec & r = g_mv_profile->recs[g_mv_profile->used++];
         r.bytes = a.M * a.row_bytes;
         r.variant = 2;
-        hipExtLaunchKernelGGL(fold_fn, dim3(FOLD_GRID), dim3(FOLD_NW * 64), smem, s, r.start, r.stop, 0, a, at, w, f, gq, seg_rows, HD);
+        hipExtLaunchKernelGGL(fold_fn, dim3(FOLD_GRID), dim3(FOLD_NW * 64), smem, s, r.start, r.stop, 0, a, at, w, f, gq, seg_rows, HD, (xblk *) pair_blocks);
         return;
     }
-    fold_fn<<<FOLD_GRID, FOLD_NW * 64, smem, s>>>(a, at, w, f, gq, seg_rows, HD);
+    fold_fn<<<FOLD_GRID, FOLD_NW * 64, smem, s>>>(a, at, w, f, gq, seg_rows, HD, (xblk *) pair_blocks);
+}
+
+__global__ void __launch_bounds__(64) attn_preq_probe_kernel(const float * x, int nb, const xblk * blocks, char * out) {
+    const int b = blockIdx.x, lane = threadIdx.x;
+    float * xc = (float *) out;
+    xblk * pub = (xblk *) (out + (size_t) nb * 256 * 4), * req = pub + nb;
+    const float4 x4 = *(const float4 *) (x + b * 256 + lane * 4);
+    *(float4 *) (xc + b * 256 + lane * 4) = x4;
+    for (int i = lane; i < XBLK_BYTES / 4; i += 64) { ((unsigned *) (pub + b))[i] = ((const unsigned *) (blocks + b))[i]; ((unsigned *) (req + b))[i] = 0u; }
+    __syncthreads();
+    const float v[4] = { x4.x, x4.y, x4.z, x4.w };
+    quantize_block_q8k(req + b, v, lane);
+}
+size_t k_attn_preq_probe_size(int64_t K) { return (size_t) K * 4 + (size_t) 2 * (K / 256) * XBLK_BYTES; }
+void k_attn_preq_probe(hipStream_t s, const float * x, int64_t K, const void * blocks, void * out) {
+    attn_preq_probe_kernel<<<(int) (K / 256), 64, 0, s>>>(x, (int) (K / 256), (const xblk *) blocks, (char *) out);
 }
 
 __global__ void __launch_bounds__(256) cross_attn_kernel(xattn_args a) {
```

Result: slower. 437.5 frames/s (-1.8%).
